# XiandaGuo/OpenStereo

Measured on NVIDIA H100. Metric: stereo_pairs_per_sec_gwcnet_256x512_d192, higher is better.
Workload: dtype f32

## Files before the change

### openstereo_b200/csrc/conv3d_tcdc.cu

```cuda
#include "tc_common.cuh"

namespace osb {

struct TcdcParams {
  const float* x;
  const void* w;
  const float* scale;
  const float* shift;
  const float* residual;
  float* y;
  int B, D, H, Cin;
  int act;
  float kappa;
  unsigned int* overflow;
  int out_ndhwc, res_ndhwc;
  int items, hblocks;
  int Wr, ctiles;
  int ystride;
  int cout_real;
};

template <int COUT, int KC, int W, int TILES, bool GW = false, int KS_ = 3>
struct TcdcCfg {
  static_assert(!GW || W == 128, "general-width tiles are 128-column segments of one input row");
  static_assert(KS_ == 3 || (KS_ == 4 && !GW), "kernel size 3 (any width) or 4 (whole-row tiles)");
  static constexpr int KS = KS_;
  static constexpr int HALO = GW ? 1 : 0;
  static constexpr int CSTEP = 128 - HALO;
  static constexpr int R = 128 / W;
  static constexpr int ROWB = KC * 4;
  static constexpr int UNIT_BYTES = 128 * ROWB;
  static constexpr int N3 = KS_ * COUT;
  static constexpr int G = 32;
  static constexpr int NG = COUT / G;
  static constexpr int NGK = KS_ * G;
  static constexpr int B_SLICE = N3 * ROWB;
  static constexpr int B_SUB = NGK * ROWB;
  static constexpr int SCOLS = KS_ == 3 ? NGK : 2 * G;
  static constexpr int LD = SCOLS + 4;
  static constexpr int NU = KS_ - 1;
  static constexpr int NLW = 4;
  static constexpr int XCHG_FLOATS = 2 * 4 * 2 * 32;
  static constexpr int FIXED_SMEM = 1024 + TC_BSLOTS * KS_ * B_SUB + TC_WGS * 128 * LD * 4 + 1024 + TC_WGS * XCHG_FLOATS * 4 + 3 * COUT * 4;
  static constexpr int STAGES = (232448 - FIXED_SMEM) / UNIT_BYTES < 10 ? (232448 - FIXED_SMEM) / UNIT_BYTES : 10;
  static_assert(STAGES >= NLW, "the ring must hold at least one unit per loader warp");
  static constexpr int HBLK = TILES * R;
  static constexpr int KSTEPS = KC / 16;
  static constexpr int LO = KC / 8;
  static constexpr int A_OFF = 0;
  static constexpr int B_OFF = A_OFF + STAGES * UNIT_BYTES;
  static constexpr int STAGE_OFF = B_OFF + TC_BSLOTS * KS_ * B_SUB;
  static constexpr int BAR_OFF = STAGE_OFF + TC_WGS * 128 * LD * 4;
  static constexpr int THREADS = TC_WG_THREADS;
  static constexpr size_t SMEM = 1024 + (size_t)BAR_OFF + 1024 + TC_WGS * XCHG_FLOATS * 4 + 3 * COUT * 4;
  static_assert(SMEM <= 232448, "shared memory budget of one CTA exceeded");
  static_assert(TILES == 1, "a consumer warpgroup holds one accumulator tile");
  static_assert(COUT % G == 0, "output channels come in groups of 32");
  static_assert(32 * LD >= TP_WARP_FLOATS, "store_ndhwc_chunk32 transposes through the warp's own rows of the staging tile");
  static_assert(B_SUB % 1024 == 0 && UNIT_BYTES % 1024 == 0, "operand tiles must stay 1024-byte aligned");
  static constexpr int kh_of(int u, int t) { return (t - 1 + 2 * u >= 0 && t - 1 + 2 * u < KS_) ? t - 1 + 2 * u : -1; }
};

struct ItemDc {
  int b, od, j0, ct, nkd;
};
__device__ __forceinline__ bool kd_valid(int od, int kd, int D) {
  const int num = od + 1 - kd;
  return !(num & 1) && num >= 0 && (num >> 1) < D;
}
__device__ __forceinline__ bool kh_valid(int ph, int kh) { return ((ph + 1 - kh) & 1) == 0; }
template <class C>
__device__ __forceinline__ ItemDc decode_dc(const TcdcParams& p, int it) {
  ItemDc w;
  w.ct = 0;
  if (C::HALO) {
    w.ct = it % p.ctiles;
    it /= p.ctiles;
  }
  const int Do = 2 * p.D;
  w.od = it % Do;
  it /= Do;
  w.j0 = (it % p.hblocks) * C::HBLK;
  w.b = it / p.hblocks;
  w.nkd = 0;
#pragma unroll
  for (int k = 0; k < C::KS; ++k) w.nkd += kd_valid(w.od, k, p.D) ? 1 : 0;
  return w;
}

template <int N, int GA, int GB, bool ADD>
__device__ __forceinline__ void dc_stage_pair(float* stage, int ld, const float (&acc)[2][N / 2], int wq, int lane) {
#pragma unroll
  for (int h = 0; h < 2; ++h) {
    float* r0 = stage + (64 * h + 16 * wq + (lane >> 2)) * ld + 2 * (lane & 3);
#pragma unroll
    for (int g = 0; g < 2; ++g)
#pragma unroll
      for (int jj = 0; jj < 4; ++jj) {
        const int j = (g ? GB : GA) * 4 + jj;
#pragma unroll
        for (int r = 0; r < 2; ++r) {
          float2* d = reinterpret_cast<float2*>(r0 + 8 * r * ld + 32 * g + 8 * jj);
          float2 v = make_float2(acc[h][4 * j + 2 * r], acc[h][4 * j + 2 * r + 1]);
          if (ADD) {
            const float2 s = *d;
            v = make_float2(s.x + v.x, s.y + v.y);
          }
          *d = v;
        }
      }
  }
}

template <int COUT, int KC, int W, int TILES, bool GW = false, int KS = 3>
__global__ void __launch_bounds__(TcdcCfg<COUT, KC, W, TILES, GW, KS>::THREADS, 1) conv3d_tcdc_kernel(const TcdcParams p) {
  using C = TcdcCfg<COUT, KC, W, TILES, GW, KS>;
  extern __shared__ __align__(1024) uint8_t smem_raw[];
  uint8_t* smem = smem_raw + ((1024u - (smem_u32(smem_raw) & 1023u)) & 1023u);
  uint8_t* a_buf = smem + C::A_OFF;
  uint8_t* b_buf = smem + C::B_OFF;
  float* stage = reinterpret_cast<float*>(smem + C::STAGE_OFF);
  uint64_t* bars = reinterpret_cast<uint64_t*>(smem + C::BAR_OFF);
  uint64_t* a_ready = bars;
  uint64_t* a_empty = a_ready + C::STAGES;
  uint64_t* b_full = a_empty + C::STAGES;
  uint64_t* b_empty = b_full + TC_BSLOTS * KS;
  float* xchg = reinterpret_cast<float*>(smem + C::BAR_OFF + 1024);
  float* s_scale = xchg + TC_WGS * C::XCHG_FLOATS;
  float* s_shift = s_scale + COUT;
  float* zeros = s_shift + COUT;

  const int warp = threadIdx.x >> 5, lane = threadIdx.x & 31;
  const int nchunk = p.Cin / KC;
  const int Wp = GW ? p.Wr : W;
  const int YS = (W < 32 && p.ystride) ? p.ystride : COUT;

  if (threadIdx.x == 0) {
    for (int s = 0; s < C::STAGES; ++s) {
      mbar_init(&a_ready[s], 32);
      mbar_init(&a_empty[s], 4 * TC_WGS);
    }
    for (int k = 0; k < TC_BSLOTS * KS; ++k) {
      mbar_init(&b_full[k], 1);
      mbar_init(&b_empty[k], 4 * TC_WGS);
    }
    fence_mbar_init();
  }
  for (int c = threadIdx.x; c < COUT; c += blockDim.x) {
    s_scale[c] = p.scale ? p.scale[c] : 1.f;
    s_shift[c] = p.shift ? p.shift[c] : 0.f;
    zeros[c] = 0.f;
  }
  __syncthreads();

  if (warp < 4 * TC_WGS) {
    setmaxnreg_inc<TC_CONSUMER_REGS>();
    const int wg = warp >> 2;
    stage += wg * 128 * C::LD;
    xchg += wg * C::XCHG_FLOATS;
    const int bar_stage = 1 + 2 * wg, bar_xchg = 2 + 2 * wg;
    const uint64_t dbase = (KC == 32) ? desc_sw128_base() : desc_sw64_base();
    constexpr uint32_t A_HALF = 64 * C::ROWB / 16;
    const uint32_t b16 = (smem_u32(b_buf) & 0x3FFFF) >> 4;
    const int q = warp & 3;
    const int m = q * 32 + lane;
    const int rr = m / W, wcol = m % W;
    const bool has_right_q = (((q + 1) * 32) % W) != 0;
    const bool has_left_q = ((q * 32) % W) != 0;
    const int Do = 2 * p.D, Ho = 2 * p.H;
    const int Wo = 2 * Wp;
    uint32_t unitc = 0, phc = 0, exc = 0;
    for (int it = blockIdx.x; it < p.items; it += gridDim.x) {
      const int cg = (it % C::NG) * C::G;
      const ItemDc w = decode_dc<C>(p, it / C::NG);
      float ev[32], od_[32];
      float acc[2][C::NGK / 2];
      uint32_t accum = 0;
      for (int kd = 0; kd < KS; ++kd) {
        if (!kd_valid(w.od, kd, p.D)) continue;
        for (int ch = 0; ch < nchunk; ++ch, ++phc) {
          const uint32_t bset = (phc & 1) * KS, bpar = (phc >> 1) & 1;
#pragma unroll
          for (int kh = 0; kh < KS; ++kh) {
            if (kh_valid(wg, kh)) continue;
            mbar_wait(&b_full[bset + kh], bpar);
            wg_release(&b_empty[bset + kh], lane);
          }
#pragma unroll
          for (int u = 0; u < C::NU; ++u) {
            const uint32_t slot = unitc % C::STAGES, par = (unitc / C::STAGES) & 1;
            mbar_wait(&a_ready[slot], par);
            const int kh = C::kh_of(u, wg);
            if (kh >= 0) {
              mbar_wait(&b_full[bset + kh], bpar);
              const uint64_t da0 = dbase | (uint64_t)((smem_u32(a_buf + slot * C::UNIT_BYTES) & 0x3FFFF) >> 4);
              const uint64_t db0 = dbase | (uint64_t)(b16 + ((bset + kh) * C::B_SUB) / 16);
              wg_fence();
#pragma unroll
              for (int ks = 0; ks < C::KSTEPS; ++ks)
                wg_mma_split<C::NGK>(acc, da0 + 2 * ks, A_HALF, db0 + 2 * ks, C::LO, ks > 0 ? 1u : accum);
              wg_commit();
              wg_wait_all();
              accum = 1;
              wg_release(&b_empty[bset + kh], lane);
            }
            wg_release(&a_empty[slot], lane);
            ++unitc;
          }
        }
      }
      const int j = w.j0 + rr;
      const bool live = j < p.H;
      const int oh = 2 * j + wg;
      const int col = GW ? w.ct * C::CSTEP + m : wcol;
      const bool cvalid = !GW || (m < C::CSTEP && col < Wp);
      const uint32_t vmask = GW ? __ballot_sync(0xffffffffu, cvalid) : 0xffffffffu;
      const size_t vox = (((size_t)w.b * Do + w.od) * Ho + oh) * Wo + 2 * col;
      if (live && cvalid && p.residual && p.res_ndhwc) {
        const float* rp = p.residual + vox * YS;
#pragma unroll
        for (int k = 0; k < 2 * COUT; k += 32) asm volatile("prefetch.global.L2 [%0];" ::"l"(rp + k));
      }
      const float corr = 1.f + p.kappa * (float)(w.nkd * (KS == 4 ? 2 : wg + 1) * nchunk * C::KSTEPS * 3);
      float* srow = stage + m * C::LD;
      float* xb = xchg + (exc & 1) * (4 * 2 * 32);
      ++exc;
      named_bar_sync(bar_stage, 128);
      if constexpr (KS == 3) {
        wg_stage<C::NGK>(stage, C::LD, acc, q, lane);
        named_bar_sync(bar_stage, 128);
        if (lane == 0) {
#pragma unroll
          for (int i = 0; i < 32; i += 4)
            *reinterpret_cast<float4*>(xb + (q * 2) * 32 + i) = *reinterpret_cast<const float4*>(srow + 2 * C::G + i);
        }
        named_bar_sync(bar_xchg, 128);
        const float* xr = has_right_q ? xb + ((q + 1) * 2) * 32 : zeros;
#pragma unroll
        for (int i0 = 0; i0 < 32; i0 += 4) {
          const float4 r4 = *reinterpret_cast<const float4*>(xr + i0);
          const float4 e4 = *reinterpret_cast<const float4*>(srow + i0);
          const float4 p24 = *reinterpret_cast<const float4*>(srow + C::G + i0);
          const float4 p04 = *reinterpret_cast<const float4*>(srow + 2 * C::G + i0);
          const float re[4] = {r4.x, r4.y, r4.z, r4.w};
          const float e[4] = {e4.x, e4.y, e4.z, e4.w}, p2[4] = {p24.x, p24.y, p24.z, p24.w}, p0[4] = {p04.x, p04.y, p04.z, p04.w};
#pragma unroll
          for (int k = 0; k < 4; ++k) {
            const int i = i0 + k;
            float right = __shfl_down_sync(0xffffffffu, p0[k], 1);
            right = (lane == 31) ? re[k] : right;
            if (W < 32) right = (wcol == W - 1) ? 0.f : right;
            ev[i] = e[k] * corr;
            od_[i] = (p2[k] + right) * corr;
          }
        }
      } else {
        dc_stage_pair<C::NGK, 1, 3, false>(stage, C::LD, acc, q, lane);
        named_bar_sync(bar_stage, 128);
        if (lane == 31) {
#pragma unroll
          for (int i = 0; i < 32; i += 4)
            *reinterpret_cast<float4*>(xb + (q * 2 + 1) * 32 + i) = *reinterpret_cast<const float4*>(srow + i);
        }
        if (lane == 0) {
#pragma unroll
          for (int i = 0; i < 32; i += 4)
            *reinterpret_cast<float4*>(xb + (q * 2) * 32 + i) = *reinterpret_cast<const float4*>(srow + C::G + i);
        }
        named_bar_sync(bar_xchg, 128);
        const float* xl = has_left_q ? xb + ((q - 1) * 2 + 1) * 32 : zeros;
        const float* xr = has_right_q ? xb + ((q + 1) * 2) * 32 : zeros;
#pragma unroll
        for (int i0 = 0; i0 < 32; i0 += 4) {
          const float4 l4 = *reinterpret_cast<const float4*>(xl + i0);
          const float4 r4 = *reinterpret_cast<const float4*>(xr + i0);
          const float4 p34 = *reinterpret_cast<const float4*>(srow + i0);
          const float4 p04 = *reinterpret_cast<const float4*>(srow + C::G + i0);
          const float le[4] = {l4.x, l4.y, l4.z, l4.w}, re[4] = {r4.x, r4.y, r4.z, r4.w};
          const float p3[4] = {p34.x, p34.y, p34.z, p34.w}, p0[4] = {p04.x, p04.y, p04.z, p04.w};
          float e[4], o[4];
#pragma unroll
          for (int k = 0; k < 4; ++k) {
            const float left = __shfl_up_sync(0xffffffffu, p3[k], 1);
            const float right = __shfl_down_sync(0xffffffffu, p0[k], 1);
            e[k] = (lane == 0) ? le[k] : left;
            o[k] = (lane == 31) ? re[k] : right;
            if (W < 32) {
              e[k] = (wcol == 0) ? 0.f : e[k];
              o[k] = (wcol == W - 1) ? 0.f : o[k];
            }
          }
          *reinterpret_cast<float4*>(srow + i0) = make_float4(e[0], e[1], e[2], e[3]);
          *reinterpret_cast<float4*>(srow + C::G + i0) = make_float4(o[0], o[1], o[2], o[3]);
        }
        named_bar_sync(bar_stage, 128);
        dc_stage_pair<C::NGK, 0, 2, true>(stage, C::LD, acc, q, lane);
        named_bar_sync(bar_stage, 128);
#pragma unroll
        for (int i0 = 0; i0 < 32; i0 += 4) {
          const float4 e4 = *reinterpret_cast<const float4*>(srow + i0);
          const float4 o4 = *reinterpret_cast<const float4*>(srow + C::G + i0);
          const float e[4] = {e4.x, e4.y, e4.z, e4.w}, o[4] = {o4.x, o4.y, o4.z, o4.w};
#pragma unroll
          for (int k = 0; k < 4; ++k) ev[i0 + k] = e[k] * corr, od_[i0 + k] = o[k] * corr;
        }
      }
      const size_t plane = (size_t)Do * Ho * Wo;
      const size_t ncdhw0 = (size_t)w.b * p.cout_real * plane + ((size_t)w.od * Ho + oh) * Wo + 2 * col;
      if (W >= 32 && live && p.out_ndhwc && (!p.residual || p.res_ndhwc)) {
        float* y0 = p.y + (vox - 2 * lane) * YS + cg;
        const float* r0 = p.residual ? p.residual + (vox - 2 * lane) * YS + cg : nullptr;
        store_ndhwc_chunk32(stage + q * 32 * C::LD, lane, ev, y0, r0, 2 * YS, s_scale + cg, s_shift + cg, p.act, vmask);
        store_ndhwc_chunk32(stage + q * 32 * C::LD, lane, od_, y0 + YS, r0 ? r0 + YS : nullptr, 2 * YS, s_scale + cg,
                            s_shift + cg, p.act, vmask);
      } else if (live && cvalid) {
#pragma unroll
        for (int i = 0; i < 32; ++i) {
          ev[i] = fmaf(ev[i], s_scale[cg + i], s_shift[cg + i]);
          od_[i] = fmaf(od_[i], s_scale[cg + i], s_shift[cg + i]);
        }
        if (p.residual) {
          if (p.res_ndhwc) {
            const float4* rp = reinterpret_cast<const float4*>(p.residual + vox * YS + cg);
            const float4* rq = reinterpret_cast<const float4*>(p.residual + (vox + 1) * YS + cg);
#pragma unroll
            for (int i = 0; i < 8; ++i) {
              const float4 a = __ldg(rp + i), bq = __ldg(rq + i);
              ev[4 * i] += a.x, ev[4 * i + 1] += a.y, ev[4 * i + 2] += a.z, ev[4 * i + 3] += a.w;
              od_[4 * i] += bq.x, od_[4 * i + 1] += bq.y, od_[4 * i + 2] += bq.z, od_[4 * i + 3] += bq.w;
            }
          } else {
#pragma unroll
            for (int i = 0; i < 32; ++i) {
              if (cg + i >= p.cout_real) continue;
              const float2 rv = __ldg(reinterpret_cast<const float2*>(p.residual + ncdhw0 + (size_t)(cg + i) * plane));
              ev[i] += rv.x, od_[i] += rv.y;
            }
          }
        }
        if (p.act == OSB_ACT_RELU) {
#pragma unroll
          for (int i = 0; i < 32; ++i) ev[i] = fmaxf(ev[i], 0.f), od_[i] = fmaxf(od_[i], 0.f);
        } else if (p.act == OSB_ACT_LEAKY) {
#pragma unroll
          for (int i = 0; i < 32; ++i) {
            ev[i] = ev[i] > 0.f ? ev[i] : 0.01f * ev[i];
            od_[i] = od_[i] > 0.f ? od_[i] : 0.01f * od_[i];
          }
        }
        if (p.out_ndhwc) {
          float4* yp = reinterpret_cast<float4*>(p.y + vox * YS + cg);
          float4* yq = reinterpret_cast<float4*>(p.y + (vox + 1) * YS + cg);
#pragma unroll
          for (int i = 0; i < 8; ++i) {
            yp[i] = make_float4(ev[4 * i], ev[4 * i + 1], ev[4 * i + 2], ev[4 * i + 3]);
            yq[i] = make_float4(od_[4 * i], od_[4 * i + 1], od_[4 * i + 2], od_[4 * i + 3]);
          }
        } else {
#pragma unroll
          for (int i = 0; i < 32; ++i)
            if (cg + i < p.cout_real) *reinterpret_cast<float2*>(p.y + ncdhw0 + (size_t)(cg + i) * plane) = make_float2(ev[i], od_[i]);
        }
      }
    }
  }
  else if (warp < 4 * TC_WGS + C::NLW) {
    setmaxnreg_dec<TC_LOADER_REGS>();
    const int lw = warp - 4 * TC_WGS;
    static_assert(KC == 16, "lane_voxel / unit-row mapping below is written for 64-byte operand rows");
    constexpr int CPR = KC / 4;
    constexpr int VPL = 32 / CPR;
    constexpr int NLD = 128 / VPL;
    static_assert(W % VPL == 0, "a load instruction must not straddle image rows");
    const int v0 = lane_voxel<KC>(lane), c = lane % CPR;
    float amax = 0.f;
    uint32_t ubase = 0;
    int first = lw;
    auto fill = [&](const float* base, size_t rstride, size_t cstride, int h_first, int h_step, uint32_t u, int col0) {
      float4 v[NLD];
#pragma unroll
      for (int j = 0; j < NLD; ++j) {
        const int hin = h_first + h_step * ((VPL * j) / W);
        const size_t off = (size_t)((VPL * j) / W) * rstride + (size_t)((VPL * j) % W) * cstride;
        bool ok = hin >= 0 && hin < p.H;
        if (GW) ok = ok && (unsigned)(col0 + VPL * j) < (unsigned)Wp;
        v[j] = ok ? __ldg(reinterpret_cast<const float4*>(base + (ptrdiff_t)off)) : make_float4(0.f, 0.f, 0.f, 0.f);
      }
      const uint32_t slot = u % C::STAGES, ph = (u / C::STAGES) & 1;
      mbar_wait_relaxed(&a_empty[slot], ph ^ 1);
      uint8_t* tile = a_buf + slot * C::UNIT_BYTES;
#pragma unroll
      for (int j = 0; j < NLD; ++j) stage_f16_split<KC>(tile, v0 + VPL * j, c, v[j], amax);
      fence_proxy_async();
      mbar_arrive(&a_ready[slot]);
    };
    for (int it = blockIdx.x; it < p.items; it += gridDim.x) {
      const ItemDc w = decode_dc<C>(p, it / C::NG);
      for (int kd = 0; kd < KS; ++kd) {
        if (!kd_valid(w.od, kd, p.D)) continue;
        const int id = (w.od + 1 - kd) >> 1;
        const float* plane = p.x + ((size_t)w.b * p.D + id) * p.H * (size_t)Wp * p.Cin;
        const int col0 = w.ct * C::CSTEP + v0;
        for (int ch = 0; ch < nchunk; ++ch) {
#pragma unroll 1
          for (int j = first; j < C::NU; j += C::NLW) {
            const int h_first = w.j0 + 1 - j;
            const float* base = plane + ((ptrdiff_t)h_first * Wp + col0) * p.Cin + ch * KC + c * 4;
            fill(base, (size_t)Wp * p.Cin, (size_t)p.Cin, h_first, 1, ubase + j, col0);
          }
          ubase += C::NU;
          first = (first + C::NLW - C::NU % C::NLW) % C::NLW;
        }
      }
    }
    tc_report_overflow(p.overflow, amax);
  }
  else {
    setmaxnreg_dec<TC_PRODUCER_REGS>();
    if (warp == 4 * TC_WGS + C::NLW && elect_one()) {
      const uint8_t* wsrc = reinterpret_cast<const uint8_t*>(p.w);
      uint32_t phc = 0;
      for (int it = blockIdx.x; it < p.items; it += gridDim.x) {
        const int cg = (it % C::NG) * C::G;
        const ItemDc w = decode_dc<C>(p, it / C::NG);
        for (int kd = 0; kd < KS; ++kd) {
          if (!kd_valid(w.od, kd, p.D)) continue;
          for (int ch = 0; ch < nchunk; ++ch, ++phc) {
            for (int kh = 0; kh < KS; ++kh) {
              const uint32_t slot = (phc & 1) * KS + kh;
              const size_t slice = ((size_t)kd * nchunk + ch) * KS + kh;
              mbar_wait_relaxed(&b_empty[slot], ((phc >> 1) & 1) ^ 1);
              mbar_arrive_expect_tx(&b_full[slot], C::B_SUB);
#pragma unroll
              for (int kw = 0; kw < KS; ++kw)
                bulk_g2s(b_buf + slot * C::B_SUB + kw * C::G * C::ROWB, wsrc + slice * C::B_SLICE + (size_t)(kw * COUT + cg) * C::ROWB,
                         C::G * C::ROWB, &b_full[slot]);
            }
          }
        }
      }
    }
    __syncwarp();
  }
}

template <int COUT, int KC, int W, int TILES, bool GW = false, int KS = 3>
static int launch_tcdc(TcdcParams& p, cudaStream_t stream) {
  using C = TcdcCfg<COUT, KC, W, TILES, GW, KS>;
  auto kernel = conv3d_tcdc_kernel<COUT, KC, W, TILES, GW, KS>;
  static PerDeviceFlag configured;
  if (!configured.here()) {
    cudaError_t e = cudaFuncSetAttribute(kernel, cudaFuncAttributeMaxDynamicSharedMemorySize, (int)C::SMEM);
    if (e != cudaSuccess) {
      set_error("conv3d_tcg: cannot reserve %zu bytes of shared memory: %s", C::SMEM, cudaGetErrorString(e));
      return OSB_ECUDA;
    }
    configured.here() = true;
  }
  if (W >= 32 && p.ystride && p.ystride != COUT) {
    set_error("conv3d_tcdc: channel slices are instantiated for W = 16 only");
    return OSB_EUNSUPPORTED;
  }
  p.hblocks = (p.H + C::HBLK - 1) / C::HBLK;
  if (p.cout_real <= 0 || p.cout_real > COUT) p.cout_real = COUT;
  if (GW) p.ctiles = (p.Wr + C::CSTEP - 1) / C::CSTEP;
  else p.Wr = W, p.ctiles = 1;
  const long long items = (long long)p.B * (2 * p.D) * p.hblocks * p.ctiles * C::NG;
  OSB_REQUIRE(items < (1ll << 31), "conv3d_tcdc: too many work items");
  p.items = (int)items;
  const int sms = sm_count();
  const int grid = (int)cap_persistent_grid(p.items < sms ? p.items : sms);
  static const std::string variant = tc_variant_name("tcdc<%d,%d,%d,%d,%d,%d>", COUT, KC, W, TILES, (int)GW, KS);
  set_tc_variant(variant.c_str());
  kernel<<<grid, C::THREADS, C::SMEM, stream>>>(p);
  count_launch();
  cudaError_t le = cudaGetLastError();
  if (le != cudaSuccess) {
    cudaFuncAttributes fa{};
    (void)cudaFuncGetAttributes(&fa, kernel);
    set_error("conv3d_tcdc_kernel<%d,%d,%d,%d>: launch failed: %s (threads %d, kernel maxThreadsPerBlock %d, regs %d, static smem %zu, "
              "dynamic smem %zu, max dynamic %d)", COUT, KC, W, TILES, cudaGetErrorString(le), C::THREADS, fa.maxThreadsPerBlock,
              fa.numRegs, fa.sharedSizeBytes, C::SMEM, fa.maxDynamicSharedSizeBytes);
    return OSB_ECUDA;
  }
  return OSB_OK;
}

}

extern "C" {

int osb_deconv3d_tc_supported(int Cin, int Cout, int W) {
  if (Cin % 16 != 0 || Cin < 16) return 0;
  if ((W == 32 && Cout == 64) || (W == 64 && Cout == 32)) return 1;
  return (osb_tc_general_width(W) && (Cout == 32 || Cout == 64)) ? 1 : 0;
}

int osb_deconv3d_k4_tc_supported(int Cin, int Cout, int W) {
  if (Cin % 16 != 0 || Cin < 16) return 0;
  return ((W == 32 && Cout == 64) || (W == 64 && Cout == 32) || (W == 16 && (Cout == 64 || Cout == 32))) ? 1 : 0;
}

static int deconv3d_k4_tc_impl(const float* x_ndhwc, const void* w_split, const float* scale, const float* shift,
                               const float* residual, float* y, int B, int Cin, int Cout, int cout_real, int D, int H, int W, int act,
                               int out_ndhwc, int res_ndhwc, int ystride, osb_stream_t stream);

int osb_deconv3d_k4_tc_fwd(const float* x_ndhwc, const void* w_split, const float* scale, const float* shift,
                           const float* residual, float* y, int B, int Cin, int Cout, int cout_real, int D, int H, int W, int act,
                           int out_ndhwc, int res_ndhwc, osb_stream_t stream) {
  return deconv3d_k4_tc_impl(x_ndhwc, w_split, scale, shift, residual, y, B, Cin, Cout, cout_real, D, H, W, act, out_ndhwc, res_ndhwc, 0,
                             stream);
}

int osb_deconv3d_k4_tc_cs_fwd(const float* x_ndhwc, const void* w_split, const float* scale, const float* shift, float* y, int B,
                              int Cin, int Cout, int D, int H, int W, int act, int ystride, osb_stream_t stream) {
  return deconv3d_k4_tc_impl(x_ndhwc, w_split, scale, shift, nullptr, y, B, Cin, Cout, Cout, D, H, W, act, 1, 1, ystride, stream);
}

static int deconv3d_k4_tc_impl(const float* x_ndhwc, const void* w_split, const float* scale, const float* shift,
                               const float* residual, float* y, int B, int Cin, int Cout, int cout_real, int D, int H, int W, int act,
                               int out_ndhwc, int res_ndhwc, int ystride, osb_stream_t stream) {
  using namespace osb;
  OSB_REQUIRE(x_ndhwc && w_split && y, "deconv3d_k4_tc: null pointer");
  OSB_REQUIRE(ystride == 0 || (ystride >= Cout && ystride % 4 == 0 && out_ndhwc && (!residual || res_ndhwc)),
              "deconv3d_k4_tc: a channel slice (ystride %d) needs channels-last tensors", ystride);
  OSB_REQUIRE(B > 0 && D > 0 && H > 0, "deconv3d_k4_tc: empty shape");
  OSB_REQUIRE(osb_deconv3d_k4_tc_supported(Cin, Cout, W), "deconv3d_k4_tc: unsupported shape Cin=%d Cout=%d W=%d", Cin, Cout, W);
  OSB_REQUIRE(act >= 0 && act <= 2, "deconv3d_k4_tc: unknown activation %d", act);
  OSB_REQUIRE(cout_real >= 1 && cout_real <= Cout && (out_ndhwc == 0 || cout_real == Cout) && (!residual || res_ndhwc == 0 || cout_real == Cout),
              "deconv3d_k4_tc: only NCDHW tensors may hold fewer (%d) channels than the packed %d", cout_real, Cout);
  TcdcParams p{};
  p.cout_real = cout_real, p.ystride = ystride;
  p.x = x_ndhwc, p.w = w_split, p.scale = scale, p.shift = shift, p.residual = residual, p.y = y;
  p.B = B, p.D = D, p.H = H, p.Cin = Cin, p.act = act, p.out_ndhwc = out_ndhwc, p.res_ndhwc = res_ndhwc;
  p.kappa = rz_kappa(), p.overflow = tc_overflow_flag();
  OSB_REQUIRE(p.overflow, "tensor-core conv: cannot allocate the overflow flag");
  cudaStream_t s = (cudaStream_t)stream;
  if (W == 16 && Cout == 64) return launch_tcdc<64, 16, 16, 1, false, 4>(p, s);
  if (W == 16 && Cout == 32) return launch_tcdc<32, 16, 16, 1, false, 4>(p, s);
  if (W == 32) return launch_tcdc<64, 16, 32, 1, false, 4>(p, s);
  return launch_tcdc<32, 16, 64, 1, false, 4>(p, s);
}

int osb_deconv3d_k3_tc_fwd(const float* x_ndhwc, const void* w_split, const float* scale, const float* shift,
                           const float* residual, float* y, int B, int Cin, int Cout, int D, int H, int W, int act,
                           int out_ndhwc, int res_ndhwc, osb_stream_t stream) {
  using namespace osb;
  OSB_REQUIRE(x_ndhwc && w_split && y, "deconv3d_k3_tc: null pointer");
  OSB_REQUIRE(B > 0 && D > 0 && H > 0, "deconv3d_k3_tc: empty shape");
  OSB_REQUIRE(osb_deconv3d_tc_supported(Cin, Cout, W), "deconv3d_k3_tc: unsupported shape Cin=%d Cout=%d W=%d", Cin, Cout, W);
  OSB_REQUIRE(act >= 0 && act <= 2, "deconv3d_k3_tc: unknown activation %d", act);
  TcdcParams p{};
  p.x = x_ndhwc, p.w = w_split, p.scale = scale, p.shift = shift, p.residual = residual, p.y = y;
  p.B = B, p.D = D, p.H = H, p.Cin = Cin, p.act = act, p.out_ndhwc = out_ndhwc, p.res_ndhwc = res_ndhwc;
  p.kappa = rz_kappa(), p.overflow = tc_overflow_flag();
  OSB_REQUIRE(p.overflow, "tensor-core conv: cannot allocate the overflow flag");
  cudaStream_t s = (cudaStream_t)stream;
  if (W == 32 && Cout == 64) return launch_tcdc<64, 16, 32, 1>(p, s);
  if (W == 64 && Cout == 32) return launch_tcdc<32, 16, 64, 1>(p, s);
  p.Wr = W;
  if (Cout == 64) return launch_tcdc<64, 16, 128, 1, true>(p, s);
  return launch_tcdc<32, 16, 128, 1, true>(p, s);
}
}
```

### openstereo_b200/csrc/conv3d_tcs2.cu

```cuda
#include "tc_common.cuh"

namespace osb {

struct Tcs2Params {
  const float* x;
  const void* w;
  const float* scale;
  const float* shift;
  const float* residual;
  float* y;
  int B, D, H, Cin;
  int act;
  float kappa;
  unsigned int* overflow;
  int out_ndhwc, res_ndhwc;
  int items, hblocks;
  int Wr, ctiles;
  int ystride;
};

template <int COUT, int KC, int W, int TILES, bool GW = false>
struct Tcs2Cfg {
  static_assert(!GW || W == 128, "general-width tiles are 128-column segments of one output row");
  static constexpr int HALO = GW ? 1 : 0;
  static constexpr int CSTEP = 128 - HALO;
  static constexpr int R = 128 / W;
  static constexpr int ROWB = KC * 4;
  static constexpr int UNIT_BYTES = 128 * ROWB;
  static constexpr int N3 = 3 * COUT;
  static constexpr int G = 32;
  static constexpr int NG = COUT / G;
  static constexpr int NP = (NG + TC_WGS - 1) / TC_WGS;
  static constexpr int B_SLICE = N3 * ROWB;
  static constexpr int B_SUB = 3 * G * ROWB;
  static constexpr int B_SLOT = TC_WGS * B_SUB;
  static constexpr int PC = 16;
  static constexpr int NPASS = G / PC;
  static constexpr int LD = 3 * PC + 4;
  static constexpr int XCHG_FLOATS = 2 * 4 * PC;
  static constexpr int NLW = 4;
  static constexpr int FIXED_SMEM = 1024 + TC_BSLOTS * 3 * B_SLOT + TC_WGS * 128 * LD * 4 + 1024 + TC_WGS * XCHG_FLOATS * 4 + 3 * COUT * 4;
  static constexpr int STAGES = (232448 - FIXED_SMEM) / UNIT_BYTES < 10 ? (232448 - FIXED_SMEM) / UNIT_BYTES : 10;
  static_assert(STAGES >= NLW, "the ring must hold at least one unit per loader warp");
  static constexpr int NU = TILES * 3 * 2;
  static constexpr int HBLK = TILES * R;
  static constexpr int KSTEPS = KC / 16;
  static constexpr int LO = KC / 8;
  static constexpr int A_OFF = 0;
  static constexpr int B_OFF = A_OFF + STAGES * UNIT_BYTES;
  static constexpr int STAGE_OFF = B_OFF + TC_BSLOTS * 3 * B_SLOT;
  static constexpr int BAR_OFF = STAGE_OFF + TC_WGS * 128 * LD * 4;
  static constexpr int THREADS = TC_WG_THREADS;
  static constexpr size_t SMEM = 1024 + (size_t)BAR_OFF + 1024 + TC_WGS * XCHG_FLOATS * 4 + 3 * COUT * 4;
  static_assert(SMEM <= 232448, "shared memory budget of one CTA exceeded");
  static_assert(TILES == 1, "a consumer warpgroup holds one accumulator tile");
  static_assert(COUT % G == 0, "output channels come in groups of 32");
  static_assert(32 * LD >= TP_WARP_FLOATS, "store_ndhwc_chunk32 transposes through the warp's own rows of the staging tile");
  static_assert(B_SUB % 1024 == 0 && UNIT_BYTES % 1024 == 0, "operand tiles must stay 1024-byte aligned");
};

template <int N>
__device__ __forceinline__ void s2_stage16(float* stage, int ld, const float (&acc)[2][N / 2], int c0, int dst, int wq, int lane) {
#pragma unroll
  for (int h = 0; h < 2; ++h) {
    float* r0 = stage + (64 * h + 16 * wq + (lane >> 2)) * ld + 2 * (lane & 3) + dst;
#pragma unroll
    for (int jj = 0; jj < 2; ++jj) {
      const int j = c0 / 8 + jj;
      *reinterpret_cast<float2*>(r0 + 8 * jj) = make_float2(acc[h][4 * j], acc[h][4 * j + 1]);
      *reinterpret_cast<float2*>(r0 + 8 * ld + 8 * jj) = make_float2(acc[h][4 * j + 2], acc[h][4 * j + 3]);
    }
  }
}

template <int COUT, int KC, int W, int TILES, bool GW = false>
__global__ void __launch_bounds__(Tcs2Cfg<COUT, KC, W, TILES, GW>::THREADS, 1) conv3d_tcs2_kernel(const Tcs2Params p) {
  using C = Tcs2Cfg<COUT, KC, W, TILES, GW>;
  extern __shared__ __align__(1024) uint8_t smem_raw[];
  uint8_t* smem = smem_raw + ((1024u - (smem_u32(smem_raw) & 1023u)) & 1023u);
  uint8_t* a_buf = smem + C::A_OFF;
  uint8_t* b_buf = smem + C::B_OFF;
  float* stage = reinterpret_cast<float*>(smem + C::STAGE_OFF);
  uint64_t* bars = reinterpret_cast<uint64_t*>(smem + C::BAR_OFF);
  uint64_t* a_ready = bars;
  uint64_t* a_empty = a_ready + C::STAGES;
  uint64_t* b_full = a_empty + C::STAGES;
  uint64_t* b_empty = b_full + TC_BSLOTS * 3;
  float* xchg = reinterpret_cast<float*>(smem + C::BAR_OFF + 1024);
  float* s_scale = xchg + TC_WGS * C::XCHG_FLOATS;
  float* s_shift = s_scale + COUT;
  float* zeros = s_shift + COUT;

  const int warp = threadIdx.x >> 5, lane = threadIdx.x & 31;
  const int nchunk = p.Cin / KC;
  const int Wp = GW ? p.Wr : W;
  const int YS = (W < 32 && p.ystride) ? p.ystride : COUT;
  const int ctiles = GW ? p.ctiles : 1;

  if (threadIdx.x == 0) {
    for (int s = 0; s < C::STAGES; ++s) {
      mbar_init(&a_ready[s], 32);
      mbar_init(&a_empty[s], 4 * TC_WGS);
    }
    for (int k = 0; k < TC_BSLOTS * 3; ++k) {
      mbar_init(&b_full[k], 1);
      mbar_init(&b_empty[k], 4 * TC_WGS);
    }
    fence_mbar_init();
  }
  for (int c = threadIdx.x; c < COUT; c += blockDim.x) {
    s_scale[c] = p.scale ? p.scale[c] : 1.f;
    s_shift[c] = p.shift ? p.shift[c] : 0.f;
    zeros[c] = 0.f;
  }
  __syncthreads();

  if (warp < 4 * TC_WGS) {
    setmaxnreg_inc<TC_CONSUMER_REGS>();
    const int wg = warp >> 2;
    stage += wg * 128 * C::LD;
    xchg += wg * C::XCHG_FLOATS;
    const int bar_stage = 1 + 2 * wg, bar_xchg = 2 + 2 * wg;
    const uint64_t dbase = (KC == 32) ? desc_sw128_base() : desc_sw64_base();
    constexpr uint32_t A_HALF = 64 * C::ROWB / 16;
    const uint32_t b16 = (smem_u32(b_buf) & 0x3FFFF) >> 4;
    const int Do = p.D / 2, Ho = p.H / 2;
    const int q = warp & 3;
    const int m = q * 32 + lane;
    const int rr = m / W, wcol = m % W;
    const bool has_left_q = ((q * 32) % W) != 0;
    uint32_t unitc = 0, phc = 0, exc = 0;
    for (int it = blockIdx.x; it < p.items; it += gridDim.x) {
      const int g = (it % C::NP) * TC_WGS + wg;
      const bool has_group = g < C::NG;
      const int cg = g * C::G;
      const int it0 = it / C::NP;
      const int ct = it0 % ctiles;
      const int hb = (it0 / ctiles) % p.hblocks;
      const int d = (it0 / (ctiles * p.hblocks)) % Do;
      const int b = it0 / (ctiles * p.hblocks * Do);
      float acc_e[2][C::G / 2], acc_o[2][C::G];
      uint32_t accum_e = 0, accum_o = 0;
      for (int kd = 0; kd < 3; ++kd) {
        const int din = 2 * d + kd - 1;
        if (din < 0 || din >= p.D) continue;
        for (int ch = 0; ch < nchunk; ++ch, ++phc) {
#pragma unroll
          for (int kh = 0; kh < 3; ++kh) {
            const uint32_t bslot = (phc & 1) * 3 + kh;
#pragma unroll
            for (int par = 0; par < 2; ++par) {
              const uint32_t slot = unitc % C::STAGES, ph = (unitc / C::STAGES) & 1;
              mbar_wait(&a_ready[slot], ph);
              if (par == 0) mbar_wait(&b_full[bslot], (phc >> 1) & 1);
              if (has_group) {
                const uint64_t da0 = dbase | (uint64_t)((smem_u32(a_buf + slot * C::UNIT_BYTES) & 0x3FFFF) >> 4);
                const uint64_t db0 = dbase | (uint64_t)(b16 + (bslot * C::B_SLOT + wg * C::B_SUB + (par ? C::G * C::ROWB : 0)) / 16);
                wg_fence();
#pragma unroll
                for (int ks = 0; ks < C::KSTEPS; ++ks) {
                  if (par == 0) wg_mma_split<C::G>(acc_e, da0 + 2 * ks, A_HALF, db0 + 2 * ks, C::LO, ks > 0 ? 1u : accum_e);
                  else wg_mma_split<2 * C::G>(acc_o, da0 + 2 * ks, A_HALF, db0 + 2 * ks, C::LO, ks > 0 ? 1u : accum_o);
                }
                wg_commit();
                wg_wait_all();
                if (par == 0) accum_e = 1;
                else accum_o = 1;
              }
              wg_release(&a_empty[slot], lane);
              if (par == 1) wg_release(&b_empty[bslot], lane);
              ++unitc;
            }
          }
        }
      }
      if (!has_group) continue;
      const int h = hb * C::HBLK + rr;
      const bool live = h < Ho;
      const int col = GW ? ct * C::CSTEP - C::HALO + m : wcol;
      const bool cvalid = !GW || (m >= C::HALO && col < Wp);
      const uint32_t vmask = GW ? __ballot_sync(0xffffffffu, cvalid) : 0xffffffffu;
      const float corr = 1.f + p.kappa * (float)(((d > 0) + 1 + (2 * d + 1 < p.D)) * nchunk * 3 * C::KSTEPS * 3);
      const ptrdiff_t vox = (((ptrdiff_t)b * Do + d) * Ho + h) * Wp + col;
      const size_t plane = (size_t)Do * Ho * Wp;
      const ptrdiff_t ncdhw0 = (ptrdiff_t)b * COUT * plane + ((ptrdiff_t)d * Ho + h) * Wp + col;
      float out[32];
#pragma unroll
      for (int pass = 0; pass < C::NPASS; ++pass) {
        named_bar_sync(bar_stage, 128);
        s2_stage16<C::G>(stage, C::LD, acc_e, pass * C::PC, 0, q, lane);
        s2_stage16<2 * C::G>(stage, C::LD, acc_o, pass * C::PC, C::PC, q, lane);
        s2_stage16<2 * C::G>(stage, C::LD, acc_o, C::G + pass * C::PC, 2 * C::PC, q, lane);
        named_bar_sync(bar_stage, 128);
        const float* srow = stage + m * C::LD;
        float* xb = xchg + (exc & 1) * (4 * C::PC);
        ++exc;
        if (lane == 31) {
#pragma unroll
          for (int i = 0; i < C::PC; i += 4)
            *reinterpret_cast<float4*>(xb + q * C::PC + i) = *reinterpret_cast<const float4*>(srow + C::PC + i);
        }
        named_bar_sync(bar_xchg, 128);
        const float* xl = has_left_q ? xb + (q - 1) * C::PC : zeros;
#pragma unroll
        for (int i0 = 0; i0 < C::PC; i0 += 4) {
          const float4 l4 = *reinterpret_cast<const float4*>(xl + i0);
          const float4 p14 = *reinterpret_cast<const float4*>(srow + i0);
          const float4 p04 = *reinterpret_cast<const float4*>(srow + C::PC + i0);
          const float4 p24 = *reinterpret_cast<const float4*>(srow + 2 * C::PC + i0);
          const float le[4] = {l4.x, l4.y, l4.z, l4.w};
          const float p0[4] = {p04.x, p04.y, p04.z, p04.w}, p1[4] = {p14.x, p14.y, p14.z, p14.w}, p2[4] = {p24.x, p24.y, p24.z, p24.w};
#pragma unroll
          for (int k = 0; k < 4; ++k) {
            float left = __shfl_up_sync(0xffffffffu, p0[k], 1);
            left = (lane == 0) ? le[k] : left;
            if (W < 32) left = (wcol == 0) ? 0.f : left;
            out[pass * C::PC + i0 + k] = ((left + p1[k]) + p2[k]) * corr;
          }
        }
      }
      const uint32_t vm = (W < 32) ? __ballot_sync(0xffffffffu, live) : (live ? vmask : 0u);
      if (vm && p.out_ndhwc && (!p.residual || p.res_ndhwc)) {
        store_ndhwc_chunk32(stage + q * 32 * C::LD, lane, out, p.y + (vox - lane) * YS + cg,
                            p.residual ? p.residual + (vox - lane) * YS + cg : nullptr, YS, s_scale + cg, s_shift + cg, p.act, vm);
      } else if (live && cvalid) {
#pragma unroll
        for (int i = 0; i < 32; ++i) out[i] = fmaf(out[i], s_scale[cg + i], s_shift[cg + i]);
        if (p.residual) {
          if (p.res_ndhwc) {
            const float4* rp = reinterpret_cast<const float4*>(p.residual + vox * YS + cg);
#pragma unroll
            for (int i = 0; i < 8; ++i) {
              const float4 rv = __ldg(rp + i);
              out[4 * i] += rv.x, out[4 * i + 1] += rv.y, out[4 * i + 2] += rv.z, out[4 * i + 3] += rv.w;
            }
          } else {
#pragma unroll
            for (int i = 0; i < 32; ++i) out[i] += __ldg(p.residual + ncdhw0 + (size_t)(cg + i) * plane);
          }
        }
        if (p.act == OSB_ACT_RELU) {
#pragma unroll
          for (int i = 0; i < 32; ++i) out[i] = fmaxf(out[i], 0.f);
        } else if (p.act == OSB_ACT_LEAKY) {
#pragma unroll
          for (int i = 0; i < 32; ++i) out[i] = out[i] > 0.f ? out[i] : 0.01f * out[i];
        }
        if (p.out_ndhwc) {
          float4* yp = reinterpret_cast<float4*>(p.y + vox * YS + cg);
#pragma unroll
          for (int i = 0; i < 8; ++i) yp[i] = make_float4(out[4 * i], out[4 * i + 1], out[4 * i + 2], out[4 * i + 3]);
        } else {
#pragma unroll
          for (int i = 0; i < 32; ++i) p.y[ncdhw0 + (size_t)(cg + i) * plane] = out[i];
        }
      }
    }
  }
  else if (warp < 4 * TC_WGS + C::NLW) {
    setmaxnreg_dec<TC_LOADER_REGS>();
    const int lw = warp - 4 * TC_WGS;
    static_assert(KC == 16, "lane_voxel / unit-row mapping below is written for 64-byte operand rows");
    constexpr int CPR = KC / 4;
    constexpr int VPL = 32 / CPR;
    constexpr int NLD = 128 / VPL;
    static_assert(W % VPL == 0, "a load instruction must not straddle image rows");
    const int v0 = lane_voxel<KC>(lane), c = lane % CPR;
    float amax = 0.f;
    const int WI = 2 * Wp;
    const int Do = p.D / 2;
    uint32_t ubase = 0;
    int first = lw;
    auto fill = [&](const float* base, size_t rstride, size_t cstride, int h_first, int h_step, uint32_t u, int col0) {
      float4 v[NLD];
#pragma unroll
      for (int j = 0; j < NLD; ++j) {
        const int hin = h_first + h_step * ((VPL * j) / W);
        const size_t off = (size_t)((VPL * j) / W) * rstride + (size_t)((VPL * j) % W) * cstride;
        bool ok = hin >= 0 && hin < p.H;
        if (GW) ok = ok && (unsigned)(col0 + VPL * j) < (unsigned)Wp;
        v[j] = ok ? __ldg(reinterpret_cast<const float4*>(base + (ptrdiff_t)off)) : make_float4(0.f, 0.f, 0.f, 0.f);
      }
      const uint32_t slot = u % C::STAGES, ph = (u / C::STAGES) & 1;
      mbar_wait_relaxed(&a_empty[slot], ph ^ 1);
      uint8_t* tile = a_buf + slot * C::UNIT_BYTES;
#pragma unroll
      for (int j = 0; j < NLD; ++j) stage_f16_split<KC>(tile, v0 + VPL * j, c, v[j], amax);
      fence_proxy_async();
      mbar_arrive(&a_ready[slot]);
    };
    for (int it = blockIdx.x; it < p.items; it += gridDim.x) {
      const int it0 = it / C::NP;
      const int ct = it0 % ctiles;
      const int hb = (it0 / ctiles) % p.hblocks;
      const int od = (it0 / (ctiles * p.hblocks)) % Do;
      const int b = it0 / (ctiles * p.hblocks * Do);
      const int h0 = hb * C::HBLK;
      const int col0 = ct * C::CSTEP - C::HALO + v0;
      for (int kd = 0; kd < 3; ++kd) {
        const int din = 2 * od + kd - 1;
        if (din < 0 || din >= p.D) continue;
        const float* plane = p.x + ((size_t)b * p.D + din) * p.H * (size_t)WI * p.Cin;
        for (int ch = 0; ch < nchunk; ++ch) {
#pragma unroll 1
          for (int j = first; j < C::NU; j += C::NLW) {
            const int t = j / 6, kh = (j >> 1) % 3, par = j & 1;
            const int h_first = 2 * (h0 + t * C::R) + kh - 1;
            const float* base = plane + ((ptrdiff_t)h_first * WI + 2 * col0 + par) * p.Cin + ch * KC + c * 4;
            fill(base, (size_t)2 * WI * p.Cin, (size_t)2 * p.Cin, h_first, 2, ubase + j, col0);
          }
          ubase += C::NU;
          first = (first + C::NLW - C::NU % C::NLW) % C::NLW;
        }
      }
    }
    tc_report_overflow(p.overflow, amax);
  }
  else {
    setmaxnreg_dec<TC_PRODUCER_REGS>();
    if (warp == 4 * TC_WGS + C::NLW && elect_one()) {
      const uint8_t* wsrc = reinterpret_cast<const uint8_t*>(p.w);
      uint32_t phc = 0;
      for (int it = blockIdx.x; it < p.items; it += gridDim.x) {
        const int g0 = (it % C::NP) * TC_WGS;
        const int ngr = min(TC_WGS, C::NG - g0);
        const int od = (it / C::NP / (ctiles * p.hblocks)) % (p.D / 2);
        for (int kd = 0; kd < 3; ++kd) {
          const int din = 2 * od + kd - 1;
          if (din < 0 || din >= p.D) continue;
          for (int ch = 0; ch < nchunk; ++ch, ++phc) {
            for (int kh = 0; kh < 3; ++kh) {
              const uint32_t slot = (phc & 1) * 3 + kh;
              const size_t slice = ((size_t)kd * nchunk + ch) * 3 + kh;
              mbar_wait_relaxed(&b_empty[slot], ((phc >> 1) & 1) ^ 1);
              mbar_arrive_expect_tx(&b_full[slot], ngr * C::B_SUB);
              for (int t = 0; t < ngr; ++t)
#pragma unroll
                for (int kw = 0; kw < 3; ++kw)
                  bulk_g2s(b_buf + slot * C::B_SLOT + t * C::B_SUB + kw * C::G * C::ROWB,
                           wsrc + slice * C::B_SLICE + (size_t)(kw * COUT + (g0 + t) * C::G) * C::ROWB, C::G * C::ROWB, &b_full[slot]);
            }
          }
        }
      }
    }
    __syncwarp();
  }
}

template <int COUT, int KC, int W, int TILES, bool GW = false>
static int launch_tcs2(Tcs2Params& p, cudaStream_t stream) {
  using C = Tcs2Cfg<COUT, KC, W, TILES, GW>;
  auto kernel = conv3d_tcs2_kernel<COUT, KC, W, TILES, GW>;
  static PerDeviceFlag configured;
  if (!configured.here()) {
    cudaError_t e = cudaFuncSetAttribute(kernel, cudaFuncAttributeMaxDynamicSharedMemorySize, (int)C::SMEM);
    if (e != cudaSuccess) {
      set_error("conv3d_tcg: cannot reserve %zu bytes of shared memory: %s", C::SMEM, cudaGetErrorString(e));
      return OSB_ECUDA;
    }
    configured.here() = true;
  }
  if (W >= 32 && p.ystride && p.ystride != COUT) {
    set_error("conv3d_tcs2: channel slices are instantiated for W = 16 only");
    return OSB_EUNSUPPORTED;
  }
  p.hblocks = (p.H / 2 + C::HBLK - 1) / C::HBLK;
  if (GW) p.ctiles = (p.Wr + C::CSTEP - 1) / C::CSTEP;
  else p.Wr = W, p.ctiles = 1;
  const long long items = (long long)p.B * (p.D / 2) * p.hblocks * p.ctiles * C::NP;
  OSB_REQUIRE(items < (1ll << 31), "conv3d_tcs2: too many work items");
  p.items = (int)items;
  const int sms = sm_count();
  const int grid = (int)cap_persistent_grid(p.items < sms ? p.items : sms);
  static const std::string variant = tc_variant_name("tcs2<%d,%d,%d,%d,%d>", COUT, KC, W, TILES, (int)GW);
  set_tc_variant(variant.c_str());
  kernel<<<grid, C::THREADS, C::SMEM, stream>>>(p);
  count_launch();
  cudaError_t le = cudaGetLastError();
  if (le != cudaSuccess) {
    cudaFuncAttributes fa{};
    (void)cudaFuncGetAttributes(&fa, kernel);
    set_error("conv3d_tcs2_kernel<%d,%d,%d,%d>: launch failed: %s (threads %d, kernel maxThreadsPerBlock %d, regs %d, static smem %zu, "
              "dynamic smem %zu, max dynamic %d)", COUT, KC, W, TILES, cudaGetErrorString(le), C::THREADS, fa.maxThreadsPerBlock,
              fa.numRegs, fa.sharedSizeBytes, C::SMEM, fa.maxDynamicSharedSizeBytes);
    return OSB_ECUDA;
  }
  return OSB_OK;
}

}

extern "C" {

int osb_conv3d_s2_tc_supported(int Cin, int Cout, int D, int H, int W) {
  if (Cin % 16 != 0 || Cin < 16 || D % 2 || H % 2 || W % 2) return 0;
  if ((W == 128 && Cout == 64) || (W == 64 && (Cout == 64 || Cout == 96 || Cout == 128)) || (W == 32 && (Cout == 64 || Cout == 96)))
    return 1;
  return (osb_tc_general_width(W / 2) && (Cout == 64 || Cout == 128)) ? 1 : 0;
}

static int conv3d_k3_s2_tc_impl(const float* x_ndhwc, const void* w_split, const float* scale, const float* shift,
                                const float* residual, float* y, int B, int Cin, int Cout, int D, int H, int W, int act,
                                int out_ndhwc, int res_ndhwc, int ystride, osb_stream_t stream) {
  using namespace osb;
  OSB_REQUIRE(ystride == 0 || (ystride >= Cout && ystride % 4 == 0 && out_ndhwc && (!residual || res_ndhwc)),
              "conv3d_k3_s2_tc: a channel slice (ystride %d) needs channels-last tensors", ystride);
  OSB_REQUIRE(x_ndhwc && w_split && y, "conv3d_k3_s2_tc: null pointer");
  OSB_REQUIRE(B > 0 && D > 0 && H > 0, "conv3d_k3_s2_tc: empty shape");
  OSB_REQUIRE(osb_conv3d_s2_tc_supported(Cin, Cout, D, H, W), "conv3d_k3_s2_tc: unsupported shape Cin=%d Cout=%d D=%d H=%d W=%d", Cin,
              Cout, D, H, W);
  OSB_REQUIRE(act >= 0 && act <= 2, "conv3d_k3_s2_tc: unknown activation %d", act);
  Tcs2Params p{};
  p.x = x_ndhwc, p.w = w_split, p.scale = scale, p.shift = shift, p.residual = residual, p.y = y;
  p.B = B, p.D = D, p.H = H, p.Cin = Cin, p.act = act, p.out_ndhwc = out_ndhwc, p.res_ndhwc = res_ndhwc;
  p.kappa = rz_kappa(), p.overflow = tc_overflow_flag();
  p.ystride = ystride;
  OSB_REQUIRE(p.overflow, "tensor-core conv: cannot allocate the overflow flag");
  cudaStream_t s = (cudaStream_t)stream;
  if (W == 32 && Cout == 96) return launch_tcs2<96, 16, 16, 1>(p, s);
  if (W == 32 && Cout == 64) return launch_tcs2<64, 16, 16, 1>(p, s);
  if (W == 128 && Cout == 64) return launch_tcs2<64, 16, 64, 1>(p, s);
  if (W == 64 && Cout == 64) return launch_tcs2<64, 16, 32, 1>(p, s);
  if (W == 64 && Cout == 128) return launch_tcs2<128, 16, 32, 1>(p, s);
  if (W == 64 && Cout == 96) return launch_tcs2<96, 16, 32, 1>(p, s);
  p.Wr = W / 2;
  if (Cout == 64) return launch_tcs2<64, 16, 128, 1, true>(p, s);
  return launch_tcs2<128, 16, 128, 1, true>(p, s);
}

int osb_conv3d_k3_s2_tc_fwd(const float* x_ndhwc, const void* w_split, const float* scale, const float* shift,
                            const float* residual, float* y, int B, int Cin, int Cout, int D, int H, int W, int act,
                            int out_ndhwc, int res_ndhwc, osb_stream_t stream) {
  return conv3d_k3_s2_tc_impl(x_ndhwc, w_split, scale, shift, residual, y, B, Cin, Cout, D, H, W, act, out_ndhwc, res_ndhwc, 0, stream);
}

int osb_conv3d_k3_s2_tc_cs_fwd(const float* x_ndhwc, const void* w_split, const float* scale, const float* shift, float* y, int B,
                               int Cin, int Cout, int D, int H, int W, int act, int ystride, osb_stream_t stream) {
  return conv3d_k3_s2_tc_impl(x_ndhwc, w_split, scale, shift, nullptr, y, B, Cin, Cout, D, H, W, act, 1, 1, ystride, stream);
}
}
```

### openstereo_b200/csrc/tc_common.cuh

```cuda
#pragma once
#include "common.cuh"

namespace osb {

__device__ __forceinline__ void mbar_wait_relaxed(uint64_t* bar, uint32_t parity) {
  uint32_t done;
  for (;;) {
    asm volatile(
        "{\n.reg .pred p;\nmbarrier.try_wait.parity.shared::cta.b64 p, [%1], %2;\nselp.u32 %0, 1, 0, p;\n}\n"
        : "=r"(done)
        : "r"(smem_u32(bar)), "r"(parity)
        : "memory");
    if (done) return;
    __nanosleep(64);
  }
}
__device__ __forceinline__ void mbar_arrive(uint64_t* bar) {
  asm volatile("mbarrier.arrive.shared::cta.b64 _, [%0];" ::"r"(smem_u32(bar)) : "memory");
}
__device__ __forceinline__ uint64_t desc_sw128_base() {
  uint64_t d = 0;
  d |= (uint64_t)1 << 16;
  d |= (uint64_t)(1024 >> 4) << 32;
  d |= (uint64_t)1 << 62;
  return d;
}
__device__ __forceinline__ uint64_t desc_sw64_base() {
  uint64_t d = 0;
  d |= (uint64_t)1 << 16;
  d |= (uint64_t)(512 >> 4) << 32;
  d |= (uint64_t)2 << 62;
  return d;
}

template <int N>
__device__ __forceinline__ void wgmma_f16(float (&d)[N / 2], uint64_t da, uint64_t db, uint32_t accumulate);
template <>
__device__ __forceinline__ void wgmma_f16<32>(float (&d)[16], uint64_t da, uint64_t db, uint32_t accumulate) {
  asm volatile(
      "{\n.reg .pred p;\nsetp.ne.b32 p, %18, 0;\n"
      "wgmma.mma_async.sync.aligned.m64n32k16.f32.f16.f16 {%0, %1, %2, %3, %4, %5, %6, %7, %8, %9, %10, %11, %12, %13, %14, %15}, %16, %17, p, 1, 1, 0, 0;\n}\n"
      : "+f"(d[0]), "+f"(d[1]), "+f"(d[2]), "+f"(d[3]), "+f"(d[4]), "+f"(d[5]), "+f"(d[6]), "+f"(d[7]), "+f"(d[8]), "+f"(d[9]), "+f"(d[10]), "+f"(d[11]), "+f"(d[12]), "+f"(d[13]), "+f"(d[14]), "+f"(d[15])
      : "l"(da), "l"(db), "r"(accumulate)
      : "memory");
}

template <>
__device__ __forceinline__ void wgmma_f16<48>(float (&d)[24], uint64_t da, uint64_t db, uint32_t accumulate) {
  asm volatile(
      "{\n.reg .pred p;\nsetp.ne.b32 p, %26, 0;\n"
      "wgmma.mma_async.sync.aligned.m64n48k16.f32.f16.f16 {%0, %1, %2, %3, %4, %5, %6, %7, %8, %9, %10, %11, %12, %13, %14, %15, %16, %17, %18, %19, %20, %21, %22, %23}, %24, %25, p, 1, 1, 0, 0;\n}\n"
      : "+f"(d[0]), "+f"(d[1]), "+f"(d[2]), "+f"(d[3]), "+f"(d[4]), "+f"(d[5]), "+f"(d[6]), "+f"(d[7]), "+f"(d[8]), "+f"(d[9]), "+f"(d[10]), "+f"(d[11]), "+f"(d[12]), "+f"(d[13]), "+f"(d[14]), "+f"(d[15]), "+f"(d[16]), "+f"(d[17]), "+f"(d[18]), "+f"(d[19]), "+f"(d[20]), "+f"(d[21]), "+f"(d[22]), "+f"(d[23])
      : "l"(da), "l"(db), "r"(accumulate)
      : "memory");
}

template <>
__device__ __forceinline__ void wgmma_f16<64>(float (&d)[32], uint64_t da, uint64_t db, uint32_t accumulate) {
  asm volatile(
      "{\n.reg .pred p;\nsetp.ne.b32 p, %34, 0;\n"
      "wgmma.mma_async.sync.aligned.m64n64k16.f32.f16.f16 {%0, %1, %2, %3, %4, %5, %6, %7, %8, %9, %10, %11, %12, %13, %14, %15, %16, %17, %18, %19, %20, %21, %22, %23, %24, %25, %26, %27, %28, %29, %30, %31}, %32, %33, p, 1, 1, 0, 0;\n}\n"
      : "+f"(d[0]), "+f"(d[1]), "+f"(d[2]), "+f"(d[3]), "+f"(d[4]), "+f"(d[5]), "+f"(d[6]), "+f"(d[7]), "+f"(d[8]), "+f"(d[9]), "+f"(d[10]), "+f"(d[11]), "+f"(d[12]), "+f"(d[13]), "+f"(d[14]), "+f"(d[15]), "+f"(d[16]), "+f"(d[17]), "+f"(d[18]), "+f"(d[19]), "+f"(d[20]), "+f"(d[21]), "+f"(d[22]), "+f"(d[23]), "+f"(d[24]), "+f"(d[25]), "+f"(d[26]), "+f"(d[27]), "+f"(d[28]), "+f"(d[29]), "+f"(d[30]), "+f"(d[31])
      : "l"(da), "l"(db), "r"(accumulate)
      : "memory");
}

template <>
__device__ __forceinline__ void wgmma_f16<96>(float (&d)[48], uint64_t da, uint64_t db, uint32_t accumulate) {
  asm volatile(
      "{\n.reg .pred p;\nsetp.ne.b32 p, %50, 0;\n"
      "wgmma.mma_async.sync.aligned.m64n96k16.f32.f16.f16 {%0, %1, %2, %3, %4, %5, %6, %7, %8, %9, %10, %11, %12, %13, %14, %15, %16, %17, %18, %19, %20, %21, %22, %23, %24, %25, %26, %27, %28, %29, %30, %31, %32, %33, %34, %35, %36, %37, %38, %39, %40, %41, %42, %43, %44, %45, %46, %47}, %48, %49, p, 1, 1, 0, 0;\n}\n"
      : "+f"(d[0]), "+f"(d[1]), "+f"(d[2]), "+f"(d[3]), "+f"(d[4]), "+f"(d[5]), "+f"(d[6]), "+f"(d[7]), "+f"(d[8]), "+f"(d[9]), "+f"(d[10]), "+f"(d[11]), "+f"(d[12]), "+f"(d[13]), "+f"(d[14]), "+f"(d[15]), "+f"(d[16]), "+f"(d[17]), "+f"(d[18]), "+f"(d[19]), "+f"(d[20]), "+f"(d[21]), "+f"(d[22]), "+f"(d[23]), "+f"(d[24]), "+f"(d[25]), "+f"(d[26]), "+f"(d[27]), "+f"(d[28]), "+f"(d[29]), "+f"(d[30]), "+f"(d[31]), "+f"(d[32]), "+f"(d[33]), "+f"(d[34]), "+f"(d[35]), "+f"(d[36]), "+f"(d[37]), "+f"(d[38]), "+f"(d[39]), "+f"(d[40]), "+f"(d[41]), "+f"(d[42]), "+f"(d[43]), "+f"(d[44]), "+f"(d[45]), "+f"(d[46]), "+f"(d[47])
      : "l"(da), "l"(db), "r"(accumulate)
      : "memory");
}

template <>
__device__ __forceinline__ void wgmma_f16<128>(float (&d)[64], uint64_t da, uint64_t db, uint32_t accumulate) {
  asm volatile(
      "{\n.reg .pred p;\nsetp.ne.b32 p, %66, 0;\n"
      "wgmma.mma_async.sync.aligned.m64n128k16.f32.f16.f16 {%0, %1, %2, %3, %4, %5, %6, %7, %8, %9, %10, %11, %12, %13, %14, %15, %16, %17, %18, %19, %20, %21, %22, %23, %24, %25, %26, %27, %28, %29, %30, %31, %32, %33, %34, %35, %36, %37, %38, %39, %40, %41, %42, %43, %44, %45, %46, %47, %48, %49, %50, %51, %52, %53, %54, %55, %56, %57, %58, %59, %60, %61, %62, %63}, %64, %65, p, 1, 1, 0, 0;\n}\n"
      : "+f"(d[0]), "+f"(d[1]), "+f"(d[2]), "+f"(d[3]), "+f"(d[4]), "+f"(d[5]), "+f"(d[6]), "+f"(d[7]), "+f"(d[8]), "+f"(d[9]), "+f"(d[10]), "+f"(d[11]), "+f"(d[12]), "+f"(d[13]), "+f"(d[14]), "+f"(d[15]), "+f"(d[16]), "+f"(d[17]), "+f"(d[18]), "+f"(d[19]), "+f"(d[20]), "+f"(d[21]), "+f"(d[22]), "+f"(d[23]), "+f"(d[24]), "+f"(d[25]), "+f"(d[26]), "+f"(d[27]), "+f"(d[28]), "+f"(d[29]), "+f"(d[30]), "+f"(d[31]), "+f"(d[32]), "+f"(d[33]), "+f"(d[34]), "+f"(d[35]), "+f"(d[36]), "+f"(d[37]), "+f"(d[38]), "+f"(d[39]), "+f"(d[40]), "+f"(d[41]), "+f"(d[42]), "+f"(d[43]), "+f"(d[44]), "+f"(d[45]), "+f"(d[46]), "+f"(d[47]), "+f"(d[48]), "+f"(d[49]), "+f"(d[50]), "+f"(d[51]), "+f"(d[52]), "+f"(d[53]), "+f"(d[54]), "+f"(d[55]), "+f"(d[56]), "+f"(d[57]), "+f"(d[58]), "+f"(d[59]), "+f"(d[60]), "+f"(d[61]), "+f"(d[62]), "+f"(d[63])
      : "l"(da), "l"(db), "r"(accumulate)
      : "memory");
}

__device__ __forceinline__ void wg_fence() { asm volatile("wgmma.fence.sync.aligned;" ::: "memory"); }
__device__ __forceinline__ void wg_commit() { asm volatile("wgmma.commit_group.sync.aligned;" ::: "memory"); }
__device__ __forceinline__ void wg_wait_all() { asm volatile("wgmma.wait_group.sync.aligned 0;" ::: "memory"); }

template <int N>
__device__ __forceinline__ void wg_mma_split(float (&acc)[2][N / 2], uint64_t da, uint32_t a_half, uint64_t db, uint32_t lo,
                                             uint32_t accumulate) {
#pragma unroll
  for (int h = 0; h < 2; ++h) {
    wgmma_f16<N>(acc[h], da + h * a_half + lo, db, accumulate);
    wgmma_f16<N>(acc[h], da + h * a_half, db + lo, 1);
    wgmma_f16<N>(acc[h], da + h * a_half, db, 1);
  }
}
__device__ __forceinline__ void wg_release(uint64_t* bar, int lane) {
  if (lane == 0) mbar_arrive(bar);
}
template <int N>
__device__ __forceinline__ void wg_stage(float* stage, int ld, const float (&acc)[2][N / 2], int wq, int lane) {
#pragma unroll
  for (int h = 0; h < 2; ++h) {
    float* r0 = stage + (64 * h + 16 * wq + (lane >> 2)) * ld + 2 * (lane & 3);
#pragma unroll
    for (int j = 0; j < N / 8; ++j) {
      *reinterpret_cast<float2*>(r0 + 8 * j) = make_float2(acc[h][4 * j], acc[h][4 * j + 1]);
      *reinterpret_cast<float2*>(r0 + 8 * ld + 8 * j) = make_float2(acc[h][4 * j + 2], acc[h][4 * j + 3]);
    }
  }
}
__device__ __forceinline__ void stage_ld16(const float* row, uint32_t* r) {
#pragma unroll
  for (int i = 0; i < 4; ++i) {
    const float4 v = reinterpret_cast<const float4*>(row)[i];
    r[4 * i] = __float_as_uint(v.x), r[4 * i + 1] = __float_as_uint(v.y), r[4 * i + 2] = __float_as_uint(v.z), r[4 * i + 3] = __float_as_uint(v.w);
  }
}

__device__ __forceinline__ void bulk_g2s(void* smem_dst, const void* gsrc, uint32_t bytes, uint64_t* bar) {
  asm volatile("cp.async.bulk.shared::cluster.global.mbarrier::complete_tx::bytes [%0], [%1], %2, [%3];" ::"r"(smem_u32(smem_dst)),
               "l"(gsrc), "r"(bytes), "r"(smem_u32(bar))
               : "memory");
}
__device__ __forceinline__ void cp_async16(void* smem_dst, const void* gsrc, bool valid) {
  const uint32_t n = valid ? 16u : 0u;
  asm volatile("cp.async.ca.shared.global [%0], [%1], 16, %2;" ::"r"(smem_u32(smem_dst)), "l"(gsrc), "r"(n) : "memory");
}
__device__ __forceinline__ void cp_async_commit() { asm volatile("cp.async.commit_group;" ::: "memory"); }
template <int N>
__device__ __forceinline__ void cp_async_wait() {
  asm volatile("cp.async.wait_group %0;" ::"n"(N) : "memory");
}
constexpr int TC_BSLOTS = 2;
__device__ __forceinline__ void named_bar_sync(int id, int threads) {
  asm volatile("bar.sync %0, %1;" ::"r"(id), "r"(threads) : "memory");
}
__device__ __forceinline__ void named_bar_arrive(int id, int threads) {
  asm volatile("bar.arrive %0, %1;" ::"r"(id), "r"(threads) : "memory");
}
constexpr int TC_WGS = 2;
constexpr int TC_CONSUMER_REGS = 184;
constexpr int TC_LOADER_REGS = 112;
constexpr int TC_PRODUCER_REGS = 32;
constexpr int TC_WG_THREADS = 512;
template <int N>
__device__ __forceinline__ void setmaxnreg_inc() {
  asm volatile("setmaxnreg.inc.sync.aligned.u32 %0;" ::"n"(N));
}
template <int N>
__device__ __forceinline__ void setmaxnreg_dec() {
  asm volatile("setmaxnreg.dec.sync.aligned.u32 %0;" ::"n"(N));
}
__device__ __forceinline__ bool elect_one() {
  uint32_t pred;
  asm volatile("{\n.reg .pred p;\nelect.sync _|p, 0xffffffff;\nselp.u32 %0, 1, 0, p;\n}\n" : "=r"(pred));
  return pred != 0;
}
constexpr float TC_ACT_SCALE = 16.f;
constexpr float TC_F16_MAX = 65504.f;
__device__ __forceinline__ uint32_t cvt_f16x2_sat(float a, float b) {
  uint32_t r;
  asm("cvt.rn.satfinite.f16x2.f32 %0, %1, %2;" : "=r"(r) : "f"(b), "f"(a));
  return r;
}
__device__ __forceinline__ float2 f16x2_to_float2(uint32_t h) {
  float2 f;
  asm("{\n.reg .b16 l, u;\nmov.b32 {l, u}, %2;\ncvt.f32.f16 %0, l;\ncvt.f32.f16 %1, u;\n}\n" : "=f"(f.x), "=f"(f.y) : "r"(h));
  return f;
}
__device__ __forceinline__ void f16_split4(const float4 v, uint2& hi, uint2& lo, float& amax) {
  const float x0 = v.x * TC_ACT_SCALE, x1 = v.y * TC_ACT_SCALE, x2 = v.z * TC_ACT_SCALE, x3 = v.w * TC_ACT_SCALE;
  amax = fmaxf(amax, fmaxf(fmaxf(fabsf(x0), fabsf(x1)), fmaxf(fabsf(x2), fabsf(x3))));
  hi.x = cvt_f16x2_sat(x0, x1);
  hi.y = cvt_f16x2_sat(x2, x3);
  const float2 h01 = f16x2_to_float2(hi.x), h23 = f16x2_to_float2(hi.y);
  lo.x = cvt_f16x2_sat(x0 - h01.x, x1 - h01.y);
  lo.y = cvt_f16x2_sat(x2 - h23.x, x3 - h23.y);
}
unsigned int* tc_overflow_flag();
__device__ __forceinline__ void tc_report_overflow(unsigned int* flag, float amax) {
  if (amax > TC_F16_MAX) atomicAdd(flag, 1u);
}

float rz_kappa();


template <int KC>
__device__ __forceinline__ int swz_offset(int row, int c) {
  if constexpr (KC == 32) return row * 128 + ((c ^ (row & 7)) << 4);
  else return row * 64 + ((c ^ ((row >> 1) & 3)) << 4);
}


template <int KC>
__device__ __forceinline__ void stage_f16_split(uint8_t* tile, int row, int q, const float4 v, float& amax) {
  uint2 hi, lo;
  f16_split4(v, hi, lo, amax);
  const int sub = (q & 1) << 3;
  *reinterpret_cast<uint2*>(tile + swz_offset<KC>(row, q >> 1) + sub) = hi;
  *reinterpret_cast<uint2*>(tile + swz_offset<KC>(row, KC / 8 + (q >> 1)) + sub) = lo;
}
template <int KC>
__device__ __forceinline__ int lane_voxel(int lane) {
  if constexpr (KC == 32) return (((lane >> 3) & 1) << 2) | (lane >> 4);
  else return ((lane >> 2) & 1) | (((lane >> 3) & 1) << 2) | ((lane >> 4) << 1);
}
template <int KC>
struct TcK {
  static constexpr int KSTEPS = KC / 16;
  static constexpr int LO_OFF = KC / 8;
};

template <int G, int DIL>
constexpr int frag_xchg_floats() { return 8 * 2 * DIL * G; }
template <int G, int DIL, int W>
__device__ __forceinline__ void frag_unshift(float (&acc)[2][3 * G / 2], float* xb, int wq, int lane, float corr, int bar) {
  constexpr int SIDE = DIL * G;
  const int l4 = lane >> 2, c0 = 2 * (lane & 3);
#pragma unroll
  for (int h = 0; h < 2; ++h) {
    float* grp = xb + (4 * h + wq) * 2 * SIDE;
    if (l4 >= 8 - DIL) {
#pragma unroll
      for (int j = 0; j < G / 8; ++j)
        *reinterpret_cast<float2*>(grp + (l4 - 8 + DIL) * G + 8 * j + c0) = make_float2(acc[h][4 * j + 2], acc[h][4 * j + 3]);
    }
    if (l4 < DIL) {
#pragma unroll
      for (int j = 0; j < G / 8; ++j)
        *reinterpret_cast<float2*>(grp + SIDE + l4 * G + 8 * j + c0) =
            make_float2(acc[h][4 * (j + G / 4)], acc[h][4 * (j + G / 4) + 1]);
    }
  }
  named_bar_sync(bar, 128);
  const int src_l = (lane - 4 * DIL) & 31, src_r = (lane + 4 * DIL) & 31;
  const bool wrap_l = l4 >= 8 - DIL, wrap_r = l4 < DIL;
#pragma unroll
  for (int h = 0; h < 2; ++h) {
    const int g = 4 * h + wq;
    const float* xl = xb + (g > 0 ? g - 1 : 0) * 2 * SIDE + (l4 < DIL ? l4 : 0) * G + c0;
    const float* xr = xb + (g < 7 ? g + 1 : 7) * 2 * SIDE + SIDE + (l4 >= 8 - DIL ? l4 - 8 + DIL : 0) * G + c0;
    const int mlo = (64 * h + 16 * wq + l4) % W, mhi = (64 * h + 16 * wq + 8 + l4) % W;
#pragma unroll
    for (int j = 0; j < G / 8; ++j) {
      const float2 sl = *reinterpret_cast<const float2*>(xl + 8 * j);
      const float2 sr = *reinterpret_cast<const float2*>(xr + 8 * j);
#pragma unroll
      for (int c2 = 0; c2 < 2; ++c2) {
        const float p0lo = acc[h][4 * j + c2], p0hi = acc[h][4 * j + 2 + c2];
        const float p2lo = acc[h][4 * (j + G / 4) + c2], p2hi = acc[h][4 * (j + G / 4) + 2 + c2];
        float llo = __shfl_sync(0xffffffffu, p0lo, src_l);
        float lhi = __shfl_sync(0xffffffffu, wrap_l ? p0lo : p0hi, src_l);
        float rlo = __shfl_sync(0xffffffffu, wrap_r ? p2hi : p2lo, src_r);
        float rhi = __shfl_sync(0xffffffffu, p2hi, src_r);
        llo = (l4 < DIL) ? (c2 ? sl.y : sl.x) : llo;
        rhi = (l4 >= 8 - DIL) ? (c2 ? sr.y : sr.x) : rhi;
        llo = (mlo < DIL) ? 0.f : llo;
        lhi = (mhi < DIL) ? 0.f : lhi;
        rlo = (mlo >= W - DIL) ? 0.f : rlo;
        rhi = (mhi >= W - DIL) ? 0.f : rhi;
        float& olo = acc[h][4 * (j + G / 8) + c2];
        float& ohi = acc[h][4 * (j + G / 8) + 2 + c2];
        olo = ((llo + olo) + rlo) * corr;
        ohi = ((lhi + ohi) + rhi) * corr;
      }
    }
  }
}
constexpr int FRAG_TP_STRIDE = 40;
constexpr int FRAG_TP_FLOATS = 16 * FRAG_TP_STRIDE;
template <int G, class Rows>
__device__ __forceinline__ void frag_epilogue(const float (&acc)[2][3 * G / 2], int lane, int wq, float* tbuf, const float* sc,
                                              const float* sh, int act, float* y, size_t ycs, const float* res, size_t rcs,
                                              const float* gate, Rows rows, int nch) {
  const int c0 = 2 * (lane & 3), l4 = lane >> 2;
  if constexpr (G == 32) {
    if (ycs == 1 && (!res || rcs == 1)) {
      const int c4 = 4 * (lane & 7), sub = lane >> 3;
      const float4 a = *reinterpret_cast<const float4*>(sc + c4);
      const float4 b = *reinterpret_cast<const float4*>(sh + c4);
#pragma unroll
      for (int h = 0; h < 2; ++h) {
        __syncwarp();
#pragma unroll
        for (int j = 0; j < 4; ++j)
#pragma unroll
          for (int rh = 0; rh < 2; ++rh)
            *reinterpret_cast<float2*>(tbuf + (8 * rh + l4) * FRAG_TP_STRIDE + 8 * j + c0) =
                make_float2(acc[h][4 * (j + 4) + 2 * rh], acc[h][4 * (j + 4) + 2 * rh + 1]);
        __syncwarp();
        float4 o[4];
        ptrdiff_t yo[4], ro[4], go[4];
        bool ok[4];
#pragma unroll
        for (int i = 0; i < 4; ++i) {
          ok[i] = rows(64 * h + 16 * wq + 4 * i + sub, yo[i], ro[i], go[i]);
          o[i] = *reinterpret_cast<const float4*>(tbuf + (4 * i + sub) * FRAG_TP_STRIDE + c4);
          o[i].x = fmaf(o[i].x, a.x, b.x), o[i].y = fmaf(o[i].y, a.y, b.y), o[i].z = fmaf(o[i].z, a.z, b.z), o[i].w = fmaf(o[i].w, a.w, b.w);
        }
        if (res) {
          float4 r[4];
#pragma unroll
          for (int i = 0; i < 4; ++i) r[i] = ok[i] ? __ldg(reinterpret_cast<const float4*>(res + ro[i] + c4)) : make_float4(0.f, 0.f, 0.f, 0.f);
#pragma unroll
          for (int i = 0; i < 4; ++i) o[i].x += r[i].x, o[i].y += r[i].y, o[i].z += r[i].z, o[i].w += r[i].w;
        }
        if (act == OSB_ACT_RELU) {
#pragma unroll
          for (int i = 0; i < 4; ++i) o[i].x = fmaxf(o[i].x, 0.f), o[i].y = fmaxf(o[i].y, 0.f), o[i].z = fmaxf(o[i].z, 0.f), o[i].w = fmaxf(o[i].w, 0.f);
        } else if (act == OSB_ACT_LEAKY) {
#pragma unroll
          for (int i = 0; i < 4; ++i) {
            o[i].x = o[i].x > 0.f ? o[i].x : 0.01f * o[i].x, o[i].y = o[i].y > 0.f ? o[i].y : 0.01f * o[i].y;
            o[i].z = o[i].z > 0.f ? o[i].z : 0.01f * o[i].z, o[i].w = o[i].w > 0.f ? o[i].w : 0.01f * o[i].w;
          }
        }
        if (gate) {
          float4 g[4];
#pragma unroll
          for (int i = 0; i < 4; ++i) g[i] = ok[i] ? __ldg(reinterpret_cast<const float4*>(gate + go[i] + c4)) : make_float4(1.f, 1.f, 1.f, 1.f);
#pragma unroll
          for (int i = 0; i < 4; ++i) o[i].x *= g[i].x, o[i].y *= g[i].y, o[i].z *= g[i].z, o[i].w *= g[i].w;
        }
#pragma unroll
        for (int i = 0; i < 4; ++i)
          if (ok[i]) *reinterpret_cast<float4*>(y + yo[i] + c4) = o[i];
      }
      return;
    }
  }
#pragma unroll
  for (int h = 0; h < 2; ++h) {
    float2 rv[G / 8][2], gv[G / 8][2];
#pragma unroll
    for (int j = 0; j < G / 8; ++j)
#pragma unroll
      for (int rh = 0; rh < 2; ++rh) {
        const int c = 8 * j + c0;
        ptrdiff_t yo, ro, go;
        const bool live = rows(64 * h + 16 * wq + l4 + 8 * rh, yo, ro, go);
        rv[j][rh] = make_float2(0.f, 0.f);
        gv[j][rh] = make_float2(1.f, 1.f);
        if (res) {
          if (rcs == 1) {
            if (live) rv[j][rh] = __ldg(reinterpret_cast<const float2*>(res + ro + c));
          } else {
            if (live && c < nch) rv[j][rh].x = __ldg(res + ro + (size_t)c * rcs);
            if (live && c + 1 < nch) rv[j][rh].y = __ldg(res + ro + (size_t)(c + 1) * rcs);
          }
        }
        if (gate && live) gv[j][rh] = __ldg(reinterpret_cast<const float2*>(gate + go + c));
      }
#pragma unroll
    for (int j = 0; j < G / 8; ++j) {
      const int c = 8 * j + c0;
      const float2 a = *reinterpret_cast<const float2*>(sc + c);
      const float2 b = *reinterpret_cast<const float2*>(sh + c);
#pragma unroll
      for (int rh = 0; rh < 2; ++rh) {
        ptrdiff_t yo, ro, go;
        const bool live = rows(64 * h + 16 * wq + l4 + 8 * rh, yo, ro, go);
        float v0 = fmaf(acc[h][4 * (j + G / 8) + 2 * rh], a.x, b.x);
        float v1 = fmaf(acc[h][4 * (j + G / 8) + 2 * rh + 1], a.y, b.y);
        if (res) v0 += rv[j][rh].x, v1 += rv[j][rh].y;
        if (act == OSB_ACT_RELU) {
          v0 = fmaxf(v0, 0.f), v1 = fmaxf(v1, 0.f);
        } else if (act == OSB_ACT_LEAKY) {
          v0 = v0 > 0.f ? v0 : 0.01f * v0, v1 = v1 > 0.f ? v1 : 0.01f * v1;
        }
        if (gate) v0 *= gv[j][rh].x, v1 *= gv[j][rh].y;
        if (!live) continue;
        if (ycs == 1) {
          *reinterpret_cast<float2*>(y + yo + c) = make_float2(v0, v1);
        } else {
          if (c < nch) y[yo + (size_t)c * ycs] = v0;
          if (c + 1 < nch) y[yo + (size_t)(c + 1) * ycs] = v1;
        }
      }
    }
  }
}

constexpr int TP_STRIDE = 36;
constexpr int TP_WARP_FLOATS = 32 * TP_STRIDE;

__device__ __forceinline__ void store_ndhwc_chunk32(float* tbuf, int lane, const float (&sum)[32], float* y0, const float* res0,
                                                    size_t vstride, const float* sc, const float* sh, int act,
                                                    uint32_t vmask = 0xffffffffu, const float* gate0 = nullptr) {
  const int c4 = 4 * (lane & 7), sub = lane >> 3;
  __syncwarp();
  float4* row = reinterpret_cast<float4*>(tbuf + lane * TP_STRIDE);
#pragma unroll
  for (int i = 0; i < 8; ++i) row[i] = make_float4(sum[4 * i], sum[4 * i + 1], sum[4 * i + 2], sum[4 * i + 3]);
  __syncwarp();
  const float4 a = *reinterpret_cast<const float4*>(sc + c4);
  const float4 b = *reinterpret_cast<const float4*>(sh + c4);
  float4 o[8];
#pragma unroll
  for (int j = 0; j < 8; ++j) {
    o[j] = *reinterpret_cast<const float4*>(tbuf + (4 * j + sub) * TP_STRIDE + c4);
    o[j].x = fmaf(o[j].x, a.x, b.x), o[j].y = fmaf(o[j].y, a.y, b.y), o[j].z = fmaf(o[j].z, a.z, b.z), o[j].w = fmaf(o[j].w, a.w, b.w);
  }
  if (res0) {
    float4 r[8];
#pragma unroll
    for (int j = 0; j < 8; ++j)
      r[j] = ((vmask >> (4 * j + sub)) & 1u) ? __ldg(reinterpret_cast<const float4*>(res0 + (size_t)(4 * j + sub) * vstride + c4))
                                             : make_float4(0.f, 0.f, 0.f, 0.f);
#pragma unroll
    for (int j = 0; j < 8; ++j) o[j].x += r[j].x, o[j].y += r[j].y, o[j].z += r[j].z, o[j].w += r[j].w;
  }
  if (act == OSB_ACT_RELU) {
#pragma unroll
    for (int j = 0; j < 8; ++j) o[j].x = fmaxf(o[j].x, 0.f), o[j].y = fmaxf(o[j].y, 0.f), o[j].z = fmaxf(o[j].z, 0.f), o[j].w = fmaxf(o[j].w, 0.f);
  } else if (act == OSB_ACT_LEAKY) {
#pragma unroll
    for (int j = 0; j < 8; ++j) {
      o[j].x = o[j].x > 0.f ? o[j].x : 0.01f * o[j].x, o[j].y = o[j].y > 0.f ? o[j].y : 0.01f * o[j].y;
      o[j].z = o[j].z > 0.f ? o[j].z : 0.01f * o[j].z, o[j].w = o[j].w > 0.f ? o[j].w : 0.01f * o[j].w;
    }
  }
  if (gate0) {
#pragma unroll
    for (int j = 0; j < 8; ++j) {
      if (!((vmask >> (4 * j + sub)) & 1u)) continue;
      const float4 g = __ldg(reinterpret_cast<const float4*>(gate0 + (size_t)(4 * j + sub) * vstride + c4));
      o[j].x *= g.x, o[j].y *= g.y, o[j].z *= g.z, o[j].w *= g.w;
    }
  }
#pragma unroll
  for (int j = 0; j < 8; ++j)
    if ((vmask >> (4 * j + sub)) & 1u) *reinterpret_cast<float4*>(y0 + (size_t)(4 * j + sub) * vstride + c4) = o[j];
}

}
```

Baseline: 284.4.

## Replace shared-memory staging epilogue with register-fragment shift-add and epilogue in deconv kernels

```diff
diff --git a/openstereo_b200/csrc/conv3d_tcdc.cu b/openstereo_b200/csrc/conv3d_tcdc.cu
--- a/openstereo_b200/csrc/conv3d_tcdc.cu
+++ b/openstereo_b200/csrc/conv3d_tcdc.cu
@@ -36,12 +36,11 @@
   static constexpr int NGK = KS_ * G;
   static constexpr int B_SLICE = N3 * ROWB;
   static constexpr int B_SUB = NGK * ROWB;
-  static constexpr int SCOLS = KS_ == 3 ? NGK : 2 * G;
-  static constexpr int LD = SCOLS + 4;
   static constexpr int NU = KS_ - 1;
   static constexpr int NLW = 4;
-  static constexpr int XCHG_FLOATS = 2 * 4 * 2 * 32;
-  static constexpr int FIXED_SMEM = 1024 + TC_BSLOTS * KS_ * B_SUB + TC_WGS * 128 * LD * 4 + 1024 + TC_WGS * XCHG_FLOATS * 4 + 3 * COUT * 4;
+  static constexpr int XCHG_FLOATS = 2 * 8 * G;
+  static constexpr int FIXED_SMEM = 1024 + TC_BSLOTS * KS_ * B_SUB + 1024 + TC_WGS * XCHG_FLOATS * 4 + 4 * TC_WGS * FRAG_TP_FLOATS * 4 +
+                                    2 * COUT * 4;
   static constexpr int STAGES = (232448 - FIXED_SMEM) / UNIT_BYTES < 10 ? (232448 - FIXED_SMEM) / UNIT_BYTES : 10;
   static_assert(STAGES >= NLW, "the ring must hold at least one unit per loader warp");
   static constexpr int HBLK = TILES * R;
@@ -49,14 +48,12 @@
   static constexpr int LO = KC / 8;
   static constexpr int A_OFF = 0;
   static constexpr int B_OFF = A_OFF + STAGES * UNIT_BYTES;
-  static constexpr int STAGE_OFF = B_OFF + TC_BSLOTS * KS_ * B_SUB;
-  static constexpr int BAR_OFF = STAGE_OFF + TC_WGS * 128 * LD * 4;
+  static constexpr int BAR_OFF = B_OFF + TC_BSLOTS * KS_ * B_SUB;
   static constexpr int THREADS = TC_WG_THREADS;
-  static constexpr size_t SMEM = 1024 + (size_t)BAR_OFF + 1024 + TC_WGS * XCHG_FLOATS * 4 + 3 * COUT * 4;
+  static constexpr size_t SMEM = 1024 + (size_t)BAR_OFF + 1024 + TC_WGS * XCHG_FLOATS * 4 + 4 * TC_WGS * FRAG_TP_FLOATS * 4 + 2 * COUT * 4;
   static_assert(SMEM <= 232448, "shared memory budget of one CTA exceeded");
   static_assert(TILES == 1, "a consumer warpgroup holds one accumulator tile");
   static_assert(COUT % G == 0, "output channels come in groups of 32");
-  static_assert(32 * LD >= TP_WARP_FLOATS, "store_ndhwc_chunk32 transposes through the warp's own rows of the staging tile");
   static_assert(B_SUB % 1024 == 0 && UNIT_BYTES % 1024 == 0, "operand tiles must stay 1024-byte aligned");
   static constexpr int kh_of(int u, int t) { return (t - 1 + 2 * u >= 0 && t - 1 + 2 * u < KS_) ? t - 1 + 2 * u : -1; }
 };
@@ -88,30 +85,6 @@
   return w;
 }
 
-template <int N, int GA, int GB, bool ADD>
-__device__ __forceinline__ void dc_stage_pair(float* stage, int ld, const float (&acc)[2][N / 2], int wq, int lane) {
-#pragma unroll
-  for (int h = 0; h < 2; ++h) {
-    float* r0 = stage + (64 * h + 16 * wq + (lane >> 2)) * ld + 2 * (lane & 3);
-#pragma unroll
-    for (int g = 0; g < 2; ++g)
-#pragma unroll
-      for (int jj = 0; jj < 4; ++jj) {
-        const int j = (g ? GB : GA) * 4 + jj;
-#pragma unroll
-        for (int r = 0; r < 2; ++r) {
-          float2* d = reinterpret_cast<float2*>(r0 + 8 * r * ld + 32 * g + 8 * jj);
-          float2 v = make_float2(acc[h][4 * j + 2 * r], acc[h][4 * j + 2 * r + 1]);
-          if (ADD) {
-            const float2 s = *d;
-            v = make_float2(s.x + v.x, s.y + v.y);
-          }
-          *d = v;
-        }
-      }
-  }
-}
-
 template <int COUT, int KC, int W, int TILES, bool GW = false, int KS = 3>
 __global__ void __launch_bounds__(TcdcCfg<COUT, KC, W, TILES, GW, KS>::THREADS, 1) conv3d_tcdc_kernel(const TcdcParams p) {
   using C = TcdcCfg<COUT, KC, W, TILES, GW, KS>;
@@ -119,16 +92,15 @@
   uint8_t* smem = smem_raw + ((1024u - (smem_u32(smem_raw) & 1023u)) & 1023u);
   uint8_t* a_buf = smem + C::A_OFF;
   uint8_t* b_buf = smem + C::B_OFF;
-  float* stage = reinterpret_cast<float*>(smem + C::STAGE_OFF);
   uint64_t* bars = reinterpret_cast<uint64_t*>(smem + C::BAR_OFF);
   uint64_t* a_ready = bars;
   uint64_t* a_empty = a_ready + C::STAGES;
   uint64_t* b_full = a_empty + C::STAGES;
   uint64_t* b_empty = b_full + TC_BSLOTS * KS;
   float* xchg = reinterpret_cast<float*>(smem + C::BAR_OFF + 1024);
-  float* s_scale = xchg + TC_WGS * C::XCHG_FLOATS;
+  float* tiles = xchg + TC_WGS * C::XCHG_FLOATS;
+  float* s_scale = tiles + 4 * TC_WGS * FRAG_TP_FLOATS;
   float* s_shift = s_scale + COUT;
-  float* zeros = s_shift + COUT;
 
   const int warp = threadIdx.x >> 5, lane = threadIdx.x & 31;
   const int nchunk = p.Cin / KC;
@@ -149,31 +121,24 @@
   for (int c = threadIdx.x; c < COUT; c += blockDim.x) {
     s_scale[c] = p.scale ? p.scale[c] : 1.f;
     s_shift[c] = p.shift ? p.shift[c] : 0.f;
-    zeros[c] = 0.f;
   }
   __syncthreads();
 
   if (warp < 4 * TC_WGS) {
     setmaxnreg_inc<TC_CONSUMER_REGS>();
     const int wg = warp >> 2;
-    stage += wg * 128 * C::LD;
     xchg += wg * C::XCHG_FLOATS;
-    const int bar_stage = 1 + 2 * wg, bar_xchg = 2 + 2 * wg;
+    const int bar_xchg = 1 + wg;
     const uint64_t dbase = (KC == 32) ? desc_sw128_base() : desc_sw64_base();
     constexpr uint32_t A_HALF = 64 * C::ROWB / 16;
     const uint32_t b16 = (smem_u32(b_buf) & 0x3FFFF) >> 4;
     const int q = warp & 3;
-    const int m = q * 32 + lane;
-    const int rr = m / W, wcol = m % W;
-    const bool has_right_q = (((q + 1) * 32) % W) != 0;
-    const bool has_left_q = ((q * 32) % W) != 0;
     const int Do = 2 * p.D, Ho = 2 * p.H;
     const int Wo = 2 * Wp;
     uint32_t unitc = 0, phc = 0, exc = 0;
     for (int it = blockIdx.x; it < p.items; it += gridDim.x) {
       const int cg = (it % C::NG) * C::G;
       const ItemDc w = decode_dc<C>(p, it / C::NG);
-      float ev[32], od_[32];
       float acc[2][C::NGK / 2];
       uint32_t accum = 0;
       for (int kd = 0; kd < KS; ++kd) {
@@ -209,159 +174,49 @@
           }
         }
       }
-      const int j = w.j0 + rr;
-      const bool live = j < p.H;
-      const int oh = 2 * j + wg;
-      const int col = GW ? w.ct * C::CSTEP + m : wcol;
-      const bool cvalid = !GW || (m < C::CSTEP && col < Wp);
-      const uint32_t vmask = GW ? __ballot_sync(0xffffffffu, cvalid) : 0xffffffffu;
-      const size_t vox = (((size_t)w.b * Do + w.od) * Ho + oh) * Wo + 2 * col;
-      if (live && cvalid && p.residual && p.res_ndhwc) {
-        const float* rp = p.residual + vox * YS;
-#pragma unroll
-        for (int k = 0; k < 2 * COUT; k += 32) asm volatile("prefetch.global.L2 [%0];" ::"l"(rp + k));
+      auto even_vox = [&](int m, bool& ok) {
+        const int j = w.j0 + m / W;
+        const int col = GW ? w.ct * C::CSTEP + m : m % W;
+        ok = j < p.H && (!GW || (m < C::CSTEP && col < Wp));
+        return (((ptrdiff_t)w.b * Do + w.od) * Ho + 2 * j + wg) * Wo + 2 * col;
+      };
+      if (p.residual && p.res_ndhwc) {
+#pragma unroll
+        for (int r = 0; r < 4; ++r) {
+          bool ok;
+          const ptrdiff_t v = even_vox(64 * (r >> 1) + 16 * q + (lane >> 2) + 8 * (r & 1), ok);
+          if (ok && (lane & 3) < 2) asm volatile("prefetch.global.L2 [%0];" ::"l"(p.residual + (v + (lane & 3)) * YS + cg));
+        }
       }
       const float corr = 1.f + p.kappa * (float)(w.nkd * (KS == 4 ? 2 : wg + 1) * nchunk * C::KSTEPS * 3);
-      float* srow = stage + m * C::LD;
-      float* xb = xchg + (exc & 1) * (4 * 2 * 32);
-      ++exc;
-      named_bar_sync(bar_stage, 128);
+      constexpr int OB = KS == 3 ? 1 : 2;
       if constexpr (KS == 3) {
-        wg_stage<C::NGK>(stage, C::LD, acc, q, lane);
-        named_bar_sync(bar_stage, 128);
-        if (lane == 0) {
-#pragma unroll
-          for (int i = 0; i < 32; i += 4)
-            *reinterpret_cast<float4*>(xb + (q * 2) * 32 + i) = *reinterpret_cast<const float4*>(srow + 2 * C::G + i);
-        }
-        named_bar_sync(bar_xchg, 128);
-        const float* xr = has_right_q ? xb + ((q + 1) * 2) * 32 : zeros;
-#pragma unroll
-        for (int i0 = 0; i0 < 32; i0 += 4) {
-          const float4 r4 = *reinterpret_cast<const float4*>(xr + i0);
-          const float4 e4 = *reinterpret_cast<const float4*>(srow + i0);
-          const float4 p24 = *reinterpret_cast<const float4*>(srow + C::G + i0);
-          const float4 p04 = *reinterpret_cast<const float4*>(srow + 2 * C::G + i0);
-          const float re[4] = {r4.x, r4.y, r4.z, r4.w};
-          const float e[4] = {e4.x, e4.y, e4.z, e4.w}, p2[4] = {p24.x, p24.y, p24.z, p24.w}, p0[4] = {p04.x, p04.y, p04.z, p04.w};
-#pragma unroll
-          for (int k = 0; k < 4; ++k) {
-            const int i = i0 + k;
-            float right = __shfl_down_sync(0xffffffffu, p0[k], 1);
-            right = (lane == 31) ? re[k] : right;
-            if (W < 32) right = (wcol == W - 1) ? 0.f : right;
-            ev[i] = e[k] * corr;
-            od_[i] = (p2[k] + right) * corr;
-          }
-        }
+        frag_shift_add<C::G, W, 1, 1, 2>(acc, acc, xchg + (exc & 1) * (C::XCHG_FLOATS / 2), q, lane, bar_xchg);
+        ++exc;
       } else {
-        dc_stage_pair<C::NGK, 1, 3, false>(stage, C::LD, acc, q, lane);
-        named_bar_sync(bar_stage, 128);
-        if (lane == 31) {
-#pragma unroll
-          for (int i = 0; i < 32; i += 4)
-            *reinterpret_cast<float4*>(xb + (q * 2 + 1) * 32 + i) = *reinterpret_cast<const float4*>(srow + i);
-        }
-        if (lane == 0) {
-#pragma unroll
-          for (int i = 0; i < 32; i += 4)
-            *reinterpret_cast<float4*>(xb + (q * 2) * 32 + i) = *reinterpret_cast<const float4*>(srow + C::G + i);
-        }
-        named_bar_sync(bar_xchg, 128);
-        const float* xl = has_left_q ? xb + ((q - 1) * 2 + 1) * 32 : zeros;
-        const float* xr = has_right_q ? xb + ((q + 1) * 2) * 32 : zeros;
-#pragma unroll
-        for (int i0 = 0; i0 < 32; i0 += 4) {
-          const float4 l4 = *reinterpret_cast<const float4*>(xl + i0);
-          const float4 r4 = *reinterpret_cast<const float4*>(xr + i0);
-          const float4 p34 = *reinterpret_cast<const float4*>(srow + i0);
-          const float4 p04 = *reinterpret_cast<const float4*>(srow + C::G + i0);
-          const float le[4] = {l4.x, l4.y, l4.z, l4.w}, re[4] = {r4.x, r4.y, r4.z, r4.w};
-          const float p3[4] = {p34.x, p34.y, p34.z, p34.w}, p0[4] = {p04.x, p04.y, p04.z, p04.w};
-          float e[4], o[4];
-#pragma unroll
-          for (int k = 0; k < 4; ++k) {
-            const float left = __shfl_up_sync(0xffffffffu, p3[k], 1);
-            const float right = __shfl_down_sync(0xffffffffu, p0[k], 1);
-            e[k] = (lane == 0) ? le[k] : left;
-            o[k] = (lane == 31) ? re[k] : right;
-            if (W < 32) {
-              e[k] = (wcol == 0) ? 0.f : e[k];
-              o[k] = (wcol == W - 1) ? 0.f : o[k];
-            }
-          }
-          *reinterpret_cast<float4*>(srow + i0) = make_float4(e[0], e[1], e[2], e[3]);
-          *reinterpret_cast<float4*>(srow + C::G + i0) = make_float4(o[0], o[1], o[2], o[3]);
-        }
-        named_bar_sync(bar_stage, 128);
-        dc_stage_pair<C::NGK, 0, 2, true>(stage, C::LD, acc, q, lane);
-        named_bar_sync(bar_stage, 128);
-#pragma unroll
-        for (int i0 = 0; i0 < 32; i0 += 4) {
-          const float4 e4 = *reinterpret_cast<const float4*>(srow + i0);
-          const float4 o4 = *reinterpret_cast<const float4*>(srow + C::G + i0);
-          const float e[4] = {e4.x, e4.y, e4.z, e4.w}, o[4] = {o4.x, o4.y, o4.z, o4.w};
-#pragma unroll
-          for (int k = 0; k < 4; ++k) ev[i0 + k] = e[k] * corr, od_[i0 + k] = o[k] * corr;
-        }
-      }
+        frag_shift_add<C::G, W, -1, 0, 1>(acc, acc, xchg + (exc & 1) * (C::XCHG_FLOATS / 2), q, lane, bar_xchg);
+        ++exc;
+        frag_shift_add<C::G, W, 1, 2, 3>(acc, acc, xchg + (exc & 1) * (C::XCHG_FLOATS / 2), q, lane, bar_xchg);
+        ++exc;
+      }
+#pragma unroll
+      for (int h = 0; h < 2; ++h)
+#pragma unroll
+        for (int i = 0; i < C::G / 2; ++i) acc[h][i] *= corr, acc[h][OB * C::G / 2 + i] *= corr;
       const size_t plane = (size_t)Do * Ho * Wo;
-      const size_t ncdhw0 = (size_t)w.b * p.cout_real * plane + ((size_t)w.od * Ho + oh) * Wo + 2 * col;
-      if (W >= 32 && live && p.out_ndhwc && (!p.residual || p.res_ndhwc)) {
-        float* y0 = p.y + (vox - 2 * lane) * YS + cg;
-        const float* r0 = p.residual ? p.residual + (vox - 2 * lane) * YS + cg : nullptr;
-        store_ndhwc_chunk32(stage + q * 32 * C::LD, lane, ev, y0, r0, 2 * YS, s_scale + cg, s_shift + cg, p.act, vmask);
-        store_ndhwc_chunk32(stage + q * 32 * C::LD, lane, od_, y0 + YS, r0 ? r0 + YS : nullptr, 2 * YS, s_scale + cg,
-                            s_shift + cg, p.act, vmask);
-      } else if (live && cvalid) {
-#pragma unroll
-        for (int i = 0; i < 32; ++i) {
-          ev[i] = fmaf(ev[i], s_scale[cg + i], s_shift[cg + i]);
-          od_[i] = fmaf(od_[i], s_scale[cg + i], s_shift[cg + i]);
-        }
-        if (p.residual) {
-          if (p.res_ndhwc) {
-            const float4* rp = reinterpret_cast<const float4*>(p.residual + vox * YS + cg);
-            const float4* rq = reinterpret_cast<const float4*>(p.residual + (vox + 1) * YS + cg);
-#pragma unroll
-            for (int i = 0; i < 8; ++i) {
-              const float4 a = __ldg(rp + i), bq = __ldg(rq + i);
-              ev[4 * i] += a.x, ev[4 * i + 1] += a.y, ev[4 * i + 2] += a.z, ev[4 * i + 3] += a.w;
-              od_[4 * i] += bq.x, od_[4 * i + 1] += bq.y, od_[4 * i + 2] += bq.z, od_[4 * i + 3] += bq.w;
-            }
-          } else {
-#pragma unroll
-            for (int i = 0; i < 32; ++i) {
-              if (cg + i >= p.cout_real) continue;
-              const float2 rv = __ldg(reinterpret_cast<const float2*>(p.residual + ncdhw0 + (size_t)(cg + i) * plane));
-              ev[i] += rv.x, od_[i] += rv.y;
-            }
-          }
-        }
-        if (p.act == OSB_ACT_RELU) {
-#pragma unroll
-          for (int i = 0; i < 32; ++i) ev[i] = fmaxf(ev[i], 0.f), od_[i] = fmaxf(od_[i], 0.f);
-        } else if (p.act == OSB_ACT_LEAKY) {
-#pragma unroll
-          for (int i = 0; i < 32; ++i) {
-            ev[i] = ev[i] > 0.f ? ev[i] : 0.01f * ev[i];
-            od_[i] = od_[i] > 0.f ? od_[i] : 0.01f * od_[i];
-          }
-        }
-        if (p.out_ndhwc) {
-          float4* yp = reinterpret_cast<float4*>(p.y + vox * YS + cg);
-          float4* yq = reinterpret_cast<float4*>(p.y + (vox + 1) * YS + cg);
-#pragma unroll
-          for (int i = 0; i < 8; ++i) {
-            yp[i] = make_float4(ev[4 * i], ev[4 * i + 1], ev[4 * i + 2], ev[4 * i + 3]);
-            yq[i] = make_float4(od_[4 * i], od_[4 * i + 1], od_[4 * i + 2], od_[4 * i + 3]);
-          }
-        } else {
-#pragma unroll
-          for (int i = 0; i < 32; ++i)
-            if (cg + i < p.cout_real) *reinterpret_cast<float2*>(p.y + ncdhw0 + (size_t)(cg + i) * plane) = make_float2(ev[i], od_[i]);
-        }
-      }
+      auto rows = [&](int m, ptrdiff_t& yo, ptrdiff_t& ro, ptrdiff_t& go) {
+        bool ok;
+        const ptrdiff_t v = even_vox(m & 127, ok) + (m >> 7);
+        const ptrdiff_t n = v + (ptrdiff_t)w.b * (p.cout_real - 1) * (ptrdiff_t)plane;
+        yo = p.out_ndhwc ? v * YS : n;
+        ro = p.res_ndhwc ? v * YS : n;
+        go = 0;
+        return ok;
+      };
+      frag_epilogue<C::G, 0, 2, OB>(acc, lane, q, tiles + warp * FRAG_TP_FLOATS, s_scale + cg, s_shift + cg, p.act,
+                                    p.y + (p.out_ndhwc ? (size_t)cg : cg * plane), p.out_ndhwc ? 1 : plane,
+                                    p.residual ? p.residual + (p.res_ndhwc ? (size_t)cg : cg * plane) : nullptr,
+                                    p.res_ndhwc ? 1 : plane, nullptr, rows, p.cout_real - cg);
     }
   }
   else if (warp < 4 * TC_WGS + C::NLW) {
diff --git a/openstereo_b200/csrc/conv3d_tcs2.cu b/openstereo_b200/csrc/conv3d_tcs2.cu
--- a/openstereo_b200/csrc/conv3d_tcs2.cu
+++ b/openstereo_b200/csrc/conv3d_tcs2.cu
@@ -34,12 +34,10 @@
   static constexpr int B_SLICE = N3 * ROWB;
   static constexpr int B_SUB = 3 * G * ROWB;
   static constexpr int B_SLOT = TC_WGS * B_SUB;
-  static constexpr int PC = 16;
-  static constexpr int NPASS = G / PC;
-  static constexpr int LD = 3 * PC + 4;
-  static constexpr int XCHG_FLOATS = 2 * 4 * PC;
+  static constexpr int XCHG_FLOATS = 2 * 8 * G;
   static constexpr int NLW = 4;
-  static constexpr int FIXED_SMEM = 1024 + TC_BSLOTS * 3 * B_SLOT + TC_WGS * 128 * LD * 4 + 1024 + TC_WGS * XCHG_FLOATS * 4 + 3 * COUT * 4;
+  static constexpr int FIXED_SMEM = 1024 + TC_BSLOTS * 3 * B_SLOT + 1024 + TC_WGS * XCHG_FLOATS * 4 + 4 * TC_WGS * FRAG_TP_FLOATS * 4 +
+                                    2 * COUT * 4;
   static constexpr int STAGES = (232448 - FIXED_SMEM) / UNIT_BYTES < 10 ? (232448 - FIXED_SMEM) / UNIT_BYTES : 10;
   static_assert(STAGES >= NLW, "the ring must hold at least one unit per loader warp");
   static constexpr int NU = TILES * 3 * 2;
@@ -48,30 +46,14 @@
   static constexpr int LO = KC / 8;
   static constexpr int A_OFF = 0;
   static constexpr int B_OFF = A_OFF + STAGES * UNIT_BYTES;
-  static constexpr int STAGE_OFF = B_OFF + TC_BSLOTS * 3 * B_SLOT;
-  static constexpr int BAR_OFF = STAGE_OFF + TC_WGS * 128 * LD * 4;
+  static constexpr int BAR_OFF = B_OFF + TC_BSLOTS * 3 * B_SLOT;
   static constexpr int THREADS = TC_WG_THREADS;
-  static constexpr size_t SMEM = 1024 + (size_t)BAR_OFF + 1024 + TC_WGS * XCHG_FLOATS * 4 + 3 * COUT * 4;
+  static constexpr size_t SMEM = 1024 + (size_t)BAR_OFF + 1024 + TC_WGS * XCHG_FLOATS * 4 + 4 * TC_WGS * FRAG_TP_FLOATS * 4 + 2 * COUT * 4;
   static_assert(SMEM <= 232448, "shared memory budget of one CTA exceeded");
   static_assert(TILES == 1, "a consumer warpgroup holds one accumulator tile");
   static_assert(COUT % G == 0, "output channels come in groups of 32");
-  static_assert(32 * LD >= TP_WARP_FLOATS, "store_ndhwc_chunk32 transposes through the warp's own rows of the staging tile");
   static_assert(B_SUB % 1024 == 0 && UNIT_BYTES % 1024 == 0, "operand tiles must stay 1024-byte aligned");
 };
-
-template <int N>
-__device__ __forceinline__ void s2_stage16(float* stage, int ld, const float (&acc)[2][N / 2], int c0, int dst, int wq, int lane) {
-#pragma unroll
-  for (int h = 0; h < 2; ++h) {
-    float* r0 = stage + (64 * h + 16 * wq + (lane >> 2)) * ld + 2 * (lane & 3) + dst;
-#pragma unroll
-    for (int jj = 0; jj < 2; ++jj) {
-      const int j = c0 / 8 + jj;
-      *reinterpret_cast<float2*>(r0 + 8 * jj) = make_float2(acc[h][4 * j], acc[h][4 * j + 1]);
-      *reinterpret_cast<float2*>(r0 + 8 * ld + 8 * jj) = make_float2(acc[h][4 * j + 2], acc[h][4 * j + 3]);
-    }
-  }
-}
 
 template <int COUT, int KC, int W, int TILES, bool GW = false>
 __global__ void __launch_bounds__(Tcs2Cfg<COUT, KC, W, TILES, GW>::THREADS, 1) conv3d_tcs2_kernel(const Tcs2Params p) {
@@ -80,16 +62,15 @@
   uint8_t* smem = smem_raw + ((1024u - (smem_u32(smem_raw) & 1023u)) & 1023u);
   uint8_t* a_buf = smem + C::A_OFF;
   uint8_t* b_buf = smem + C::B_OFF;
-  float* stage = reinterpret_cast<float*>(smem + C::STAGE_OFF);
   uint64_t* bars = reinterpret_cast<uint64_t*>(smem + C::BAR_OFF);
   uint64_t* a_ready = bars;
   uint64_t* a_empty = a_ready + C::STAGES;
   uint64_t* b_full = a_empty + C::STAGES;
   uint64_t* b_empty = b_full + TC_BSLOTS * 3;
   float* xchg = reinterpret_cast<float*>(smem + C::BAR_OFF + 1024);
-  float* s_scale = xchg + TC_WGS * C::XCHG_FLOATS;
+  float* tiles = xchg + TC_WGS * C::XCHG_FLOATS;
+  float* s_scale = tiles + 4 * TC_WGS * FRAG_TP_FLOATS;
   float* s_shift = s_scale + COUT;
-  float* zeros = s_shift + COUT;
 
   const int warp = threadIdx.x >> 5, lane = threadIdx.x & 31;
   const int nchunk = p.Cin / KC;
@@ -111,24 +92,19 @@
   for (int c = threadIdx.x; c < COUT; c += blockDim.x) {
     s_scale[c] = p.scale ? p.scale[c] : 1.f;
     s_shift[c] = p.shift ? p.shift[c] : 0.f;
-    zeros[c] = 0.f;
   }
   __syncthreads();
 
   if (warp < 4 * TC_WGS) {
     setmaxnreg_inc<TC_CONSUMER_REGS>();
     const int wg = warp >> 2;
-    stage += wg * 128 * C::LD;
     xchg += wg * C::XCHG_FLOATS;
-    const int bar_stage = 1 + 2 * wg, bar_xchg = 2 + 2 * wg;
+    const int bar_xchg = 1 + wg;
     const uint64_t dbase = (KC == 32) ? desc_sw128_base() : desc_sw64_base();
     constexpr uint32_t A_HALF = 64 * C::ROWB / 16;
     const uint32_t b16 = (smem_u32(b_buf) & 0x3FFFF) >> 4;
     const int Do = p.D / 2, Ho = p.H / 2;
     const int q = warp & 3;
-    const int m = q * 32 + lane;
-    const int rr = m / W, wcol = m % W;
-    const bool has_left_q = ((q * 32) % W) != 0;
     uint32_t unitc = 0, phc = 0, exc = 0;
     for (int it = blockIdx.x; it < p.items; it += gridDim.x) {
       const int g = (it % C::NP) * TC_WGS + wg;
@@ -175,86 +151,28 @@
         }
       }
       if (!has_group) continue;
-      const int h = hb * C::HBLK + rr;
-      const bool live = h < Ho;
-      const int col = GW ? ct * C::CSTEP - C::HALO + m : wcol;
-      const bool cvalid = !GW || (m >= C::HALO && col < Wp);
-      const uint32_t vmask = GW ? __ballot_sync(0xffffffffu, cvalid) : 0xffffffffu;
       const float corr = 1.f + p.kappa * (float)(((d > 0) + 1 + (2 * d + 1 < p.D)) * nchunk * 3 * C::KSTEPS * 3);
-      const ptrdiff_t vox = (((ptrdiff_t)b * Do + d) * Ho + h) * Wp + col;
+      frag_shift_add<C::G, W, -1, 0, 0>(acc_e, acc_o, xchg + (exc & 1) * (C::XCHG_FLOATS / 2), q, lane, bar_xchg);
+      ++exc;
+#pragma unroll
+      for (int hh = 0; hh < 2; ++hh)
+#pragma unroll
+        for (int i = 0; i < C::G / 2; ++i) acc_e[hh][i] = (acc_e[hh][i] + acc_o[hh][C::G / 2 + i]) * corr;
       const size_t plane = (size_t)Do * Ho * Wp;
-      const ptrdiff_t ncdhw0 = (ptrdiff_t)b * COUT * plane + ((ptrdiff_t)d * Ho + h) * Wp + col;
-      float out[32];
-#pragma unroll
-      for (int pass = 0; pass < C::NPASS; ++pass) {
-        named_bar_sync(bar_stage, 128);
-        s2_stage16<C::G>(stage, C::LD, acc_e, pass * C::PC, 0, q, lane);
-        s2_stage16<2 * C::G>(stage, C::LD, acc_o, pass * C::PC, C::PC, q, lane);
-        s2_stage16<2 * C::G>(stage, C::LD, acc_o, C::G + pass * C::PC, 2 * C::PC, q, lane);
-        named_bar_sync(bar_stage, 128);
-        const float* srow = stage + m * C::LD;
-        float* xb = xchg + (exc & 1) * (4 * C::PC);
-        ++exc;
-        if (lane == 31) {
-#pragma unroll
-          for (int i = 0; i < C::PC; i += 4)
-            *reinterpret_cast<float4*>(xb + q * C::PC + i) = *reinterpret_cast<const float4*>(srow + C::PC + i);
-        }
-        named_bar_sync(bar_xchg, 128);
-        const float* xl = has_left_q ? xb + (q - 1) * C::PC : zeros;
-#pragma unroll
-        for (int i0 = 0; i0 < C::PC; i0 += 4) {
-          const float4 l4 = *reinterpret_cast<const float4*>(xl + i0);
-          const float4 p14 = *reinterpret_cast<const float4*>(srow + i0);
-          const float4 p04 = *reinterpret_cast<const float4*>(srow + C::PC + i0);
-          const float4 p24 = *reinterpret_cast<const float4*>(srow + 2 * C::PC + i0);
-          const float le[4] = {l4.x, l4.y, l4.z, l4.w};
-          const float p0[4] = {p04.x, p04.y, p04.z, p04.w}, p1[4] = {p14.x, p14.y, p14.z, p14.w}, p2[4] = {p24.x, p24.y, p24.z, p24.w};
-#pragma unroll
-          for (int k = 0; k < 4; ++k) {
-            float left = __shfl_up_sync(0xffffffffu, p0[k], 1);
-            left = (lane == 0) ? le[k] : left;
-            if (W < 32) left = (wcol == 0) ? 0.f : left;
-            out[pass * C::PC + i0 + k] = ((left + p1[k]) + p2[k]) * corr;
-          }
-        }
-      }
-      const uint32_t vm = (W < 32) ? __ballot_sync(0xffffffffu, live) : (live ? vmask : 0u);
-      if (vm && p.out_ndhwc && (!p.residual || p.res_ndhwc)) {
-        store_ndhwc_chunk32(stage + q * 32 * C::LD, lane, out, p.y + (vox - lane) * YS + cg,
-                            p.residual ? p.residual + (vox - lane) * YS + cg : nullptr, YS, s_scale + cg, s_shift + cg, p.act, vm);
-      } else if (live && cvalid) {
-#pragma unroll
-        for (int i = 0; i < 32; ++i) out[i] = fmaf(out[i], s_scale[cg + i], s_shift[cg + i]);
-        if (p.residual) {
-          if (p.res_ndhwc) {
-            const float4* rp = reinterpret_cast<const float4*>(p.residual + vox * YS + cg);
-#pragma unroll
-            for (int i = 0; i < 8; ++i) {
-              const float4 rv = __ldg(rp + i);
-              out[4 * i] += rv.x, out[4 * i + 1] += rv.y, out[4 * i + 2] += rv.z, out[4 * i + 3] += rv.w;
-            }
-          } else {
-#pragma unroll
-            for (int i = 0; i < 32; ++i) out[i] += __ldg(p.residual + ncdhw0 + (size_t)(cg + i) * plane);
-          }
-        }
-        if (p.act == OSB_ACT_RELU) {
-#pragma unroll
-          for (int i = 0; i < 32; ++i) out[i] = fmaxf(out[i], 0.f);
-        } else if (p.act == OSB_ACT_LEAKY) {
-#pragma unroll
-          for (int i = 0; i < 32; ++i) out[i] = out[i] > 0.f ? out[i] : 0.01f * out[i];
-        }
-        if (p.out_ndhwc) {
-          float4* yp = reinterpret_cast<float4*>(p.y + vox * YS + cg);
-#pragma unroll
-          for (int i = 0; i < 8; ++i) yp[i] = make_float4(out[4 * i], out[4 * i + 1], out[4 * i + 2], out[4 * i + 3]);
-        } else {
-#pragma unroll
-          for (int i = 0; i < 32; ++i) p.y[ncdhw0 + (size_t)(cg + i) * plane] = out[i];
-        }
-      }
+      auto rows = [&](int m, ptrdiff_t& yo, ptrdiff_t& ro, ptrdiff_t& go) {
+        const int h = hb * C::HBLK + m / W;
+        const int col = GW ? ct * C::CSTEP - C::HALO + m : m % W;
+        const ptrdiff_t v = (((ptrdiff_t)b * Do + d) * Ho + h) * Wp + col;
+        const ptrdiff_t n = v + (ptrdiff_t)b * (COUT - 1) * (ptrdiff_t)plane;
+        yo = p.out_ndhwc ? v * YS : n;
+        ro = p.res_ndhwc ? v * YS : n;
+        go = 0;
+        return h < Ho && (!GW || (m >= C::HALO && col < Wp));
+      };
+      frag_epilogue<C::G, 0>(acc_e, lane, q, tiles + warp * FRAG_TP_FLOATS, s_scale + cg, s_shift + cg, p.act,
+                             p.y + (p.out_ndhwc ? (size_t)cg : cg * plane), p.out_ndhwc ? 1 : plane,
+                             p.residual ? p.residual + (p.res_ndhwc ? (size_t)cg : cg * plane) : nullptr, p.res_ndhwc ? 1 : plane,
+                             nullptr, rows, C::G);
     }
   }
   else if (warp < 4 * TC_WGS + C::NLW) {
diff --git a/openstereo_b200/csrc/tc_common.cuh b/openstereo_b200/csrc/tc_common.cuh
--- a/openstereo_b200/csrc/tc_common.cuh
+++ b/openstereo_b200/csrc/tc_common.cuh
@@ -101,25 +101,6 @@
 }
 __device__ __forceinline__ void wg_release(uint64_t* bar, int lane) {
   if (lane == 0) mbar_arrive(bar);
-}
-template <int N>
-__device__ __forceinline__ void wg_stage(float* stage, int ld, const float (&acc)[2][N / 2], int wq, int lane) {
-#pragma unroll
-  for (int h = 0; h < 2; ++h) {
-    float* r0 = stage + (64 * h + 16 * wq + (lane >> 2)) * ld + 2 * (lane & 3);
-#pragma unroll
-    for (int j = 0; j < N / 8; ++j) {
-      *reinterpret_cast<float2*>(r0 + 8 * j) = make_float2(acc[h][4 * j], acc[h][4 * j + 1]);
-      *reinterpret_cast<float2*>(r0 + 8 * ld + 8 * j) = make_float2(acc[h][4 * j + 2], acc[h][4 * j + 3]);
-    }
-  }
-}
-__device__ __forceinline__ void stage_ld16(const float* row, uint32_t* r) {
-#pragma unroll
-  for (int i = 0; i < 4; ++i) {
-    const float4 v = reinterpret_cast<const float4*>(row)[i];
-    r[4 * i] = __float_as_uint(v.x), r[4 * i + 1] = __float_as_uint(v.y), r[4 * i + 2] = __float_as_uint(v.z), r[4 * i + 3] = __float_as_uint(v.w);
-  }
 }
 
 __device__ __forceinline__ void bulk_g2s(void* smem_dst, const void* gsrc, uint32_t bytes, uint64_t* bar) {
@@ -272,10 +253,59 @@
     }
   }
 }
+template <int G, int W, int DIR, int DB, int SB, int ND, int NS>
+__device__ __forceinline__ void frag_shift_add(float (&dst)[2][ND], const float (&src)[2][NS], float* xb, int wq, int lane, int bar) {
+  static_assert(DIR == -1 || DIR == 1, "one row to the left or to the right");
+  const int l4 = lane >> 2, c0 = 2 * (lane & 3);
+  if (l4 == (DIR < 0 ? 7 : 0)) {
+#pragma unroll
+    for (int h = 0; h < 2; ++h)
+#pragma unroll
+      for (int j = 0; j < G / 8; ++j) {
+        const int r = 4 * (j + SB * G / 8) + (DIR < 0 ? 2 : 0);
+        *reinterpret_cast<float2*>(xb + (4 * h + wq) * G + 8 * j + c0) = make_float2(src[h][r], src[h][r + 1]);
+      }
+  }
+  named_bar_sync(bar, 128);
+  const int src_l = (lane + 4 * DIR) & 31;
+  const bool wrap = DIR < 0 ? l4 == 7 : l4 == 0;
+#pragma unroll
+  for (int h = 0; h < 2; ++h) {
+    const int g = 4 * h + wq + DIR;
+    const float* xs = xb + (g < 0 ? 0 : g > 7 ? 7 : g) * G + c0;
+    const int mlo = (64 * h + 16 * wq + l4) % W, mhi = (64 * h + 16 * wq + 8 + l4) % W;
+#pragma unroll
+    for (int j = 0; j < G / 8; ++j) {
+      const float2 sv = *reinterpret_cast<const float2*>(xs + 8 * j);
+#pragma unroll
+      for (int c2 = 0; c2 < 2; ++c2) {
+        const float slo = src[h][4 * (j + SB * G / 8) + c2], shi = src[h][4 * (j + SB * G / 8) + 2 + c2];
+        float nlo, nhi;
+        if constexpr (DIR < 0) {
+          nlo = __shfl_sync(0xffffffffu, slo, src_l);
+          nhi = __shfl_sync(0xffffffffu, wrap ? slo : shi, src_l);
+          nlo = (l4 == 0) ? (c2 ? sv.y : sv.x) : nlo;
+          nlo = (mlo == 0) ? 0.f : nlo;
+          nhi = (mhi == 0) ? 0.f : nhi;
+        } else {
+          nlo = __shfl_sync(0xffffffffu, wrap ? shi : slo, src_l);
+          nhi = __shfl_sync(0xffffffffu, shi, src_l);
+          nhi = (l4 == 7) ? (c2 ? sv.y : sv.x) : nhi;
+          nlo = (mlo == W - 1) ? 0.f : nlo;
+          nhi = (mhi == W - 1) ? 0.f : nhi;
+        }
+        float& dlo = dst[h][4 * (j + DB * G / 8) + c2];
+        float& dhi = dst[h][4 * (j + DB * G / 8) + 2 + c2];
+        dlo = nlo + dlo;
+        dhi = nhi + dhi;
+      }
+    }
+  }
+}
 constexpr int FRAG_TP_STRIDE = 40;
 constexpr int FRAG_TP_FLOATS = 16 * FRAG_TP_STRIDE;
-template <int G, class Rows>
-__device__ __forceinline__ void frag_epilogue(const float (&acc)[2][3 * G / 2], int lane, int wq, float* tbuf, const float* sc,
+template <int G, int BLK = 1, int NP = 1, int PSTRIDE = 1, int NA, class Rows>
+__device__ __forceinline__ void frag_epilogue(const float (&acc)[2][NA], int lane, int wq, float* tbuf, const float* sc,
                                               const float* sh, int act, float* y, size_t ycs, const float* res, size_t rcs,
                                               const float* gate, Rows rows, int nch) {
   const int c0 = 2 * (lane & 3), l4 = lane >> 2;
@@ -286,54 +316,64 @@
       const float4 b = *reinterpret_cast<const float4*>(sh + c4);
 #pragma unroll
       for (int h = 0; h < 2; ++h) {
-        __syncwarp();
-#pragma unroll
-        for (int j = 0; j < 4; ++j)
-#pragma unroll
-          for (int rh = 0; rh < 2; ++rh)
-            *reinterpret_cast<float2*>(tbuf + (8 * rh + l4) * FRAG_TP_STRIDE + 8 * j + c0) =
-                make_float2(acc[h][4 * (j + 4) + 2 * rh], acc[h][4 * (j + 4) + 2 * rh + 1]);
-        __syncwarp();
-        float4 o[4];
-        ptrdiff_t yo[4], ro[4], go[4];
-        bool ok[4];
-#pragma unroll
-        for (int i = 0; i < 4; ++i) {
-          ok[i] = rows(64 * h + 16 * wq + 4 * i + sub, yo[i], ro[i], go[i]);
-          o[i] = *reinterpret_cast<const float4*>(tbuf + (4 * i + sub) * FRAG_TP_STRIDE + c4);
-          o[i].x = fmaf(o[i].x, a.x, b.x), o[i].y = fmaf(o[i].y, a.y, b.y), o[i].z = fmaf(o[i].z, a.z, b.z), o[i].w = fmaf(o[i].w, a.w, b.w);
+        float4 o[4 * NP];
+        ptrdiff_t ro[4 * NP], go[4 * NP];
+        bool ok[4 * NP];
+#pragma unroll
+        for (int par = 0; par < NP; ++par) {
+          __syncwarp();
+#pragma unroll
+          for (int j = 0; j < 4; ++j)
+#pragma unroll
+            for (int rh = 0; rh < 2; ++rh)
+              *reinterpret_cast<float2*>(tbuf + (8 * rh + l4) * FRAG_TP_STRIDE + 8 * j + c0) =
+                  make_float2(acc[h][4 * (j + 4 * (BLK + par * PSTRIDE)) + 2 * rh], acc[h][4 * (j + 4 * (BLK + par * PSTRIDE)) + 2 * rh + 1]);
+          __syncwarp();
+#pragma unroll
+          for (int i = 0; i < 4; ++i) {
+            const int k = 4 * par + i;
+            ptrdiff_t yo;
+            ok[k] = rows(128 * par + 64 * h + 16 * wq + 4 * i + sub, yo, ro[k], go[k]);
+            o[k] = *reinterpret_cast<const float4*>(tbuf + (4 * i + sub) * FRAG_TP_STRIDE + c4);
+            o[k].x = fmaf(o[k].x, a.x, b.x), o[k].y = fmaf(o[k].y, a.y, b.y), o[k].z = fmaf(o[k].z, a.z, b.z), o[k].w = fmaf(o[k].w, a.w, b.w);
+          }
         }
         if (res) {
-          float4 r[4];
-#pragma unroll
-          for (int i = 0; i < 4; ++i) r[i] = ok[i] ? __ldg(reinterpret_cast<const float4*>(res + ro[i] + c4)) : make_float4(0.f, 0.f, 0.f, 0.f);
-#pragma unroll
-          for (int i = 0; i < 4; ++i) o[i].x += r[i].x, o[i].y += r[i].y, o[i].z += r[i].z, o[i].w += r[i].w;
+          float4 r[4 * NP];
+#pragma unroll
+          for (int i = 0; i < 4 * NP; ++i) r[i] = ok[i] ? __ldg(reinterpret_cast<const float4*>(res + ro[i] + c4)) : make_float4(0.f, 0.f, 0.f, 0.f);
+#pragma unroll
+          for (int i = 0; i < 4 * NP; ++i) o[i].x += r[i].x, o[i].y += r[i].y, o[i].z += r[i].z, o[i].w += r[i].w;
         }
         if (act == OSB_ACT_RELU) {
 #pragma unroll
-          for (int i = 0; i < 4; ++i) o[i].x = fmaxf(o[i].x, 0.f), o[i].y = fmaxf(o[i].y, 0.f), o[i].z = fmaxf(o[i].z, 0.f), o[i].w = fmaxf(o[i].w, 0.f);
+          for (int i = 0; i < 4 * NP; ++i) o[i].x = fmaxf(o[i].x, 0.f), o[i].y = fmaxf(o[i].y, 0.f), o[i].z = fmaxf(o[i].z, 0.f), o[i].w = fmaxf(o[i].w, 0.f);
         } else if (act == OSB_ACT_LEAKY) {
 #pragma unroll
-          for (int i = 0; i < 4; ++i) {
+          for (int i = 0; i < 4 * NP; ++i) {
             o[i].x = o[i].x > 0.f ? o[i].x : 0.01f * o[i].x, o[i].y = o[i].y > 0.f ? o[i].y : 0.01f * o[i].y;
             o[i].z = o[i].z > 0.f ? o[i].z : 0.01f * o[i].z, o[i].w = o[i].w > 0.f ? o[i].w : 0.01f * o[i].w;
           }
         }
         if (gate) {
-          float4 g[4];
-#pragma unroll
-          for (int i = 0; i < 4; ++i) g[i] = ok[i] ? __ldg(reinterpret_cast<const float4*>(gate + go[i] + c4)) : make_float4(1.f, 1.f, 1.f, 1.f);
-#pragma unroll
-          for (int i = 0; i < 4; ++i) o[i].x *= g[i].x, o[i].y *= g[i].y, o[i].z *= g[i].z, o[i].w *= g[i].w;
-        }
-#pragma unroll
-        for (int i = 0; i < 4; ++i)
-          if (ok[i]) *reinterpret_cast<float4*>(y + yo[i] + c4) = o[i];
+          float4 g[4 * NP];
+#pragma unroll
+          for (int i = 0; i < 4 * NP; ++i) g[i] = ok[i] ? __ldg(reinterpret_cast<const float4*>(gate + go[i] + c4)) : make_float4(1.f, 1.f, 1.f, 1.f);
+#pragma unroll
+          for (int i = 0; i < 4 * NP; ++i) o[i].x *= g[i].x, o[i].y *= g[i].y, o[i].z *= g[i].z, o[i].w *= g[i].w;
+        }
+#pragma unroll
+        for (int i = 0; i < 4 * NP; ++i) {
+          ptrdiff_t yo, ro_, go_;
+          rows(128 * (i / 4) + 64 * h + 16 * wq + 4 * (i % 4) + sub, yo, ro_, go_);
+          if (ok[i]) *reinterpret_cast<float4*>(y + yo + c4) = o[i];
+        }
       }
       return;
     }
   }
+#pragma unroll
+  for (int par = 0; par < NP; ++par)
 #pragma unroll
   for (int h = 0; h < 2; ++h) {
     float2 rv[G / 8][2], gv[G / 8][2];
@@ -343,7 +383,7 @@
       for (int rh = 0; rh < 2; ++rh) {
         const int c = 8 * j + c0;
         ptrdiff_t yo, ro, go;
-        const bool live = rows(64 * h + 16 * wq + l4 + 8 * rh, yo, ro, go);
+        const bool live = rows(128 * par + 64 * h + 16 * wq + l4 + 8 * rh, yo, ro, go);
         rv[j][rh] = make_float2(0.f, 0.f);
         gv[j][rh] = make_float2(1.f, 1.f);
         if (res) {
@@ -364,9 +404,9 @@
 #pragma unroll
       for (int rh = 0; rh < 2; ++rh) {
         ptrdiff_t yo, ro, go;
-        const bool live = rows(64 * h + 16 * wq + l4 + 8 * rh, yo, ro, go);
-        float v0 = fmaf(acc[h][4 * (j + G / 8) + 2 * rh], a.x, b.x);
-        float v1 = fmaf(acc[h][4 * (j + G / 8) + 2 * rh + 1], a.y, b.y);
+        const bool live = rows(128 * par + 64 * h + 16 * wq + l4 + 8 * rh, yo, ro, go);
+        float v0 = fmaf(acc[h][4 * (j + (BLK + par * PSTRIDE) * G / 8) + 2 * rh], a.x, b.x);
+        float v1 = fmaf(acc[h][4 * (j + (BLK + par * PSTRIDE) * G / 8) + 2 * rh + 1], a.y, b.y);
         if (res) v0 += rv[j][rh].x, v1 += rv[j][rh].y;
         if (act == OSB_ACT_RELU) {
           v0 = fmaxf(v0, 0.f), v1 = fmaxf(v1, 0.f);
@@ -386,56 +426,4 @@
   }
 }
 
-constexpr int TP_STRIDE = 36;
-constexpr int TP_WARP_FLOATS = 32 * TP_STRIDE;
-
-__device__ __forceinline__ void store_ndhwc_chunk32(float* tbuf, int lane, const float (&sum)[32], float* y0, const float* res0,
-                                                    size_t vstride, const float* sc, const float* sh, int act,
-                                                    uint32_t vmask = 0xffffffffu, const float* gate0 = nullptr) {
-  const int c4 = 4 * (lane & 7), sub = lane >> 3;
-  __syncwarp();
-  float4* row = reinterpret_cast<float4*>(tbuf + lane * TP_STRIDE);
-#pragma unroll
-  for (int i = 0; i < 8; ++i) row[i] = make_float4(sum[4 * i], sum[4 * i + 1], sum[4 * i + 2], sum[4 * i + 3]);
-  __syncwarp();
-  const float4 a = *reinterpret_cast<const float4*>(sc + c4);
-  const float4 b = *reinterpret_cast<const float4*>(sh + c4);
-  float4 o[8];
-#pragma unroll
-  for (int j = 0; j < 8; ++j) {
-    o[j] = *reinterpret_cast<const float4*>(tbuf + (4 * j + sub) * TP_STRIDE + c4);
-    o[j].x = fmaf(o[j].x, a.x, b.x), o[j].y = fmaf(o[j].y, a.y, b.y), o[j].z = fmaf(o[j].z, a.z, b.z), o[j].w = fmaf(o[j].w, a.w, b.w);
-  }
-  if (res0) {
-    float4 r[8];
-#pragma unroll
-    for (int j = 0; j < 8; ++j)
-      r[j] = ((vmask >> (4 * j + sub)) & 1u) ? __ldg(reinterpret_cast<const float4*>(res0 + (size_t)(4 * j + sub) * vstride + c4))
-                                             : make_float4(0.f, 0.f, 0.f, 0.f);
-#pragma unroll
-    for (int j = 0; j < 8; ++j) o[j].x += r[j].x, o[j].y += r[j].y, o[j].z += r[j].z, o[j].w += r[j].w;
-  }
-  if (act == OSB_ACT_RELU) {
-#pragma unroll
-    for (int j = 0; j < 8; ++j) o[j].x = fmaxf(o[j].x, 0.f), o[j].y = fmaxf(o[j].y, 0.f), o[j].z = fmaxf(o[j].z, 0.f), o[j].w = fmaxf(o[j].w, 0.f);
-  } else if (act == OSB_ACT_LEAKY) {
-#pragma unroll
-    for (int j = 0; j < 8; ++j) {
-      o[j].x = o[j].x > 0.f ? o[j].x : 0.01f * o[j].x, o[j].y = o[j].y > 0.f ? o[j].y : 0.01f * o[j].y;
-      o[j].z = o[j].z > 0.f ? o[j].z : 0.01f * o[j].z, o[j].w = o[j].w > 0.f ? o[j].w : 0.01f * o[j].w;
-    }
-  }
-  if (gate0) {
-#pragma unroll
-    for (int j = 0; j < 8; ++j) {
-      if (!((vmask >> (4 * j + sub)) & 1u)) continue;
-      const float4 g = __ldg(reinterpret_cast<const float4*>(gate0 + (size_t)(4 * j + sub) * vstride + c4));
-      o[j].x *= g.x, o[j].y *= g.y, o[j].z *= g.z, o[j].w *= g.w;
-    }
-  }
-#pragma unroll
-  for (int j = 0; j < 8; ++j)
-    if ((vmask >> (4 * j + sub)) & 1u) *reinterpret_cast<float4*>(y0 + (size_t)(4 * j + sub) * vstride + c4) = o[j];
-}
-
-}
+}
```

Result: no change. 284.7 (median of 6 runs) (+0.1%).
